# srinidhiPY/SSL_CR_Histo

Measured on AMD Instinct MI355X. Metric: images/sec (ResNet18 SSL_CR step, 256x256 bf16 synthetic patches; whole job), higher is better.
Workload: dtype bf16

## Files before the change

### include/sslcr.h

```cpp
#ifndef SSLCR_H_
#define SSLCR_H_
#include <stddef.h>
#include <stdint.h>

#ifdef __cplusplus
extern "C" {
#endif
#if defined(__GNUC__) || defined(__clang__)
#pragma GCC visibility push(default)
#endif

#define SSLCR_F32 0
#define SSLCR_BF16 1
#define SSLCR_FP8 2

int sslcr_version(void);
const char* sslcr_last_error(void);

typedef struct sslcr_conv_desc {
  const void* x;
  const void* w;
  void* y;
  const float* in_scale;
  const float* in_shift;
  const float* bias;
  const void* residual;
  float* stats;
  int N, H, W, C, K, R, S, stride, pad;
  int PH, PW;
  int OH, OW, osh;
  int transposed;
  int in_relu, relu, accumulate;
  int pix_mul, pix_off_h, pix_off_w;
  unsigned tap_mask;
  const void* mask_x; const float* mask_scale; const float* mask_shift; const float* mask_mean;
  int par4;
  int seg_images, seg_stride;
  const float* out_scale;
} sslcr_conv_desc;
int sslcr_conv2d(int dtype, const sslcr_conv_desc* d, void* stream);
int sslcr_conv2d_partial_rows(const sslcr_conv_desc* d);
int sslcr_conv2d_segments_ok(int dtype, const sslcr_conv_desc* d);
const char* sslcr_conv2d_kernel_name(int dtype, const sslcr_conv_desc* d);
int sslcr_conv2d_s2_pair(int dtype, const sslcr_conv_desc* c1, const sslcr_conv_desc* ds, void* stream);
int sslcr_conv2d_s2_pair_ok(int dtype, const sslcr_conv_desc* c1, const sslcr_conv_desc* ds);

typedef struct sslcr_fp8_desc {
  const uint8_t* w8;
  const float* w_dequant;
  float x_scale;
  const float* x_scale_dev;
  float* amax_out;
} sslcr_fp8_desc;
int sslcr_conv2d_fp8(const sslcr_conv_desc* d, const sslcr_fp8_desc* q, void* stream);
int sslcr_conv2d_fp8_partial_rows(const sslcr_conv_desc* d);
typedef struct sslcr_pack_fp8_desc {
  const float* w;
  uint8_t* w8;
  float* w_dequant;
  const float* gamma; const float* beta; const float* rmean; const float* rvar; float eps; float* bias_out;
  int K, C;
} sslcr_pack_fp8_desc;
int sslcr_pack_conv_fp8(const sslcr_pack_fp8_desc* d, void* stream);

typedef struct sslcr_wgrad_desc {
  const void* x;
  const void* dy;
  float* dw;
  const float* in_scale;
  const float* in_shift;
  int in_relu;
  int N, H, W, C, K, R, S, stride, pad, OH, OW;
  int seg_images;
  int seg_stride;
} sslcr_wgrad_desc;
int sslcr_conv2d_wgrad(int dtype, const sslcr_wgrad_desc* d, void* stream);
const char* sslcr_conv2d_wgrad_kernel_name(int dtype, const sslcr_wgrad_desc* d);

int sslcr_probe_tr16(const uint16_t* in, const int* byte_addr, uint16_t* out, void* stream);

typedef struct sslcr_stem_desc {
  const void* x;
  const void* w;
  void* y;
  const float* bias;
  float* stats;
  int N, H, W, OH, OW, in_f32, relu;
  const void* x2;
  int n_split;
  const float* out_scale;
} sslcr_stem_desc;
int sslcr_stem_conv(int dtype, const sslcr_stem_desc* d, void* stream);
int sslcr_stem_partial_rows(const sslcr_stem_desc* d);
int sslcr_stem_conv_pool(int dtype, const sslcr_stem_desc* d, int POH, int POW, void* stream);
typedef struct sslcr_stem_wgrad_desc {
  const void* x; const void* dy;
  float* dw;
  int N, H, W, OH, OW, in_f32;
  const void* x2; int n_split;
} sslcr_stem_wgrad_desc;
int sslcr_stem_wgrad(int dtype, const sslcr_stem_wgrad_desc* d, void* stream);

typedef struct sslcr_bn_finalize_desc {
  const float* partials;
  int rows, C;
  double count;
  const float* gamma; const float* beta;
  float* scale; float* shift; float* mean; float* invstd;
  float* running_mean; float* running_var; int64_t* num_batches_tracked;
  float momentum, eps; int replay;
  double* sums_out;
  const double* sums_in;
  double* stage;
  int nseg, seg_stride;
  int* tickets;
} sslcr_bn_finalize_desc;
int sslcr_bn_finalize(const sslcr_bn_finalize_desc* d, void* stream);

typedef struct sslcr_bn_act_desc {
  const void* x; const float* scale; const float* shift;
  const void* res; const float* rscale; const float* rshift;
  void* y; size_t pixels; int C; int relu;
  int nseg, seg_stride;
  uint8_t* ybits;
} sslcr_bn_act_desc;
// ... 192 lines not shown
```

### ssl_cr_histo_amd/_lib.py

```python
import ctypes as C
import os

import torch

HERE = os.path.dirname(os.path.abspath(__file__))
LIB_PATH = os.path.join(HERE, "libsslcr.so")

vp, i32, f32, f64, sz = C.c_void_p, C.c_int, C.c_float, C.c_double, C.c_size_t


class SslcrError(RuntimeError):
    pass


def _S(name, fields):
    return type(name, (C.Structure,), {"_fields_": fields})


ConvDesc = _S("ConvDesc", [("x", vp), ("w", vp), ("y", vp), ("in_scale", vp), ("in_shift", vp), ("bias", vp),
                           ("residual", vp), ("stats", vp)] +
              [(k, i32) for k in ("N", "H", "W", "C", "K", "R", "S", "stride", "pad", "PH", "PW", "OH", "OW", "osh",
                                  "transposed", "in_relu", "relu", "accumulate", "pix_mul", "pix_off_h", "pix_off_w")] +
              [("tap_mask", C.c_uint), ("mask_x", vp), ("mask_scale", vp), ("mask_shift", vp), ("mask_mean", vp),
               ("par4", i32), ("seg_images", i32), ("seg_stride", i32), ("out_scale", vp)])
WgradDesc = _S("WgradDesc", [("x", vp), ("dy", vp), ("dw", vp), ("in_scale", vp), ("in_shift", vp), ("in_relu", i32)] +
               [(k, i32) for k in ("N", "H", "W", "C", "K", "R", "S", "stride", "pad", "OH", "OW", "seg_images", "seg_stride")])
StemDesc = _S("StemDesc", [("x", vp), ("w", vp), ("y", vp), ("bias", vp), ("stats", vp)] +
              [(k, i32) for k in ("N", "H", "W", "OH", "OW", "in_f32", "relu")] + [("x2", vp), ("n_split", i32), ("out_scale", vp)])
StemWgradDesc = _S("StemWgradDesc", [("x", vp), ("dy", vp), ("dw", vp)] +
                   [(k, i32) for k in ("N", "H", "W", "OH", "OW", "in_f32")] + [("x2", vp), ("n_split", i32)])
BnFinalizeDesc = _S("BnFinalizeDesc", [("partials", vp), ("rows", i32), ("C", i32), ("count", f64), ("gamma", vp),
                                       ("beta", vp), ("scale", vp), ("shift", vp), ("mean", vp), ("invstd", vp),
                                       ("running_mean", vp), ("running_var", vp), ("num_batches_tracked", vp),
                                       ("momentum", f32), ("eps", f32), ("replay", i32), ("sums_out", vp),
                                       ("sums_in", vp), ("stage", vp), ("nseg", i32), ("seg_stride", i32), ("tickets", vp)])
BnActDesc = _S("BnActDesc", [("x", vp), ("scale", vp), ("shift", vp), ("res", vp), ("rscale", vp), ("rshift", vp),
                             ("y", vp), ("pixels", sz), ("C", i32), ("relu", i32), ("nseg", i32), ("seg_stride", i32), ("ybits", vp)])
PoolFwdDesc = _S("PoolFwdDesc", [("x", vp), ("scale", vp), ("shift", vp), ("y", vp), ("argmax", vp)] +
                 [(k, i32) for k in ("N", "H", "W", "C", "OH", "OW")])
PoolBwdDesc = _S("PoolBwdDesc", [("dy", vp), ("argmax", vp), ("x", vp), ("scale", vp), ("shift", vp), ("dx", vp)] +
                 [(k, i32) for k in ("N", "H", "W", "C", "OH", "OW")])
BnBwdDesc = _S("BnBwdDesc", [("dy", vp), ("x", vp), ("yact", vp), ("scale", vp), ("shift", vp), ("mean", vp),
                             ("invstd", vp), ("sums", vp), ("dx", vp), ("gout", vp), ("pixels", sz), ("C", i32),
                             ("relu_from_x", i32), ("count", f64), ("pool_dy", vp), ("pool_argmax", vp), ("pH", i32),
                             ("pW", i32), ("pOH", i32), ("pOW", i32), ("pool_y", vp), ("g_in_reduce", i32), ("dgamma", vp), ("dbeta", vp),
                             ("pg_scale", f32), ("nseg", i32), ("seg_stride", i32), ("sums_stride", i32), ("yact_bits", vp)])
LossDesc = _S("LossDesc", [("kind", i32), ("logits", vp), ("logits_t", vp), ("target_f", vp), ("target_i", vp),
                           ("dlogits", vp), ("out", vp), ("nx", i32), ("nu", i32), ("C", i32), ("lambda_u", f32),
                           ("inv_nx_global", f32), ("inv_nu_global", f32)])
TensorDesc = _S("TensorDesc", [("p", vp), ("g", vp), ("s1", vp), ("s2", vp), ("n", i32), ("K", i32), ("C", i32),
                               ("RS", i32), ("w_fwd", vp), ("w_dgrad", vp), ("pack_dtype", i32), ("dgrad_flip", i32)])
OptDesc = _S("OptDesc", [("kind", i32), ("lr", f32), ("beta1", f32), ("beta2", f32), ("eps", f32), ("wd", f32),
                         ("momentum", f32), ("bc1", f32), ("bc2", f32), ("first_step", i32), ("grad_scale", f32)])
WeakAugDesc = _S("WeakAugDesc", [("src", vp), ("dst", vp), ("params", vp)] +
                 [(k, i32) for k in ("N", "SH", "SW", "OH", "OW", "src_hwc")])
ColourAugDesc = _S("ColourAugDesc", [("src", vp), ("dst", vp), ("shift", vp), ("apply", vp), ("hed_from_rgb", f64 * 9),
                                     ("rgb_from_hed", f64 * 9), ("N", i32), ("H", i32), ("W", i32), ("hwc", i32)])
BrightnessContrastDesc = _S("BrightnessContrastDesc", [("src", vp), ("dst", vp), ("alpha_beta", vp), ("apply", vp), ("stats", vp),
                                                       ("N", i32), ("H", i32), ("W", i32)])
PackDesc = _S("PackDesc", [("w", vp), ("w_fwd", vp), ("w_dgrad", vp), ("gamma", vp), ("beta", vp), ("rmean", vp),
                           ("rvar", vp), ("eps", f32), ("bias_out", vp)] + [(k, i32) for k in ("K", "C", "R", "S", "dgrad_flip")] + [("scale_out", vp)])

Fp8Desc = _S("Fp8Desc", [("w8", vp), ("w_dequant", vp), ("x_scale", f32), ("x_scale_dev", vp), ("amax_out", vp)])
PackFp8Desc = _S("PackFp8Desc", [("w", vp), ("w8", vp), ("w_dequant", vp), ("gamma", vp), ("beta", vp), ("rmean", vp), ("rvar", vp),
                                 ("eps", f32), ("bias_out", vp), ("K", i32), ("C", i32)])

P = C.POINTER
SIGNATURES = {
    "sslcr_version": (i32, []),
    "sslcr_last_error": (C.c_char_p, []),
    "sslcr_conv2d": (i32, [i32, P(ConvDesc), vp]),
    "sslcr_conv2d_partial_rows": (i32, [P(ConvDesc)]),
    "sslcr_conv2d_segments_ok": (i32, [i32, P(ConvDesc)]),
    "sslcr_conv2d_kernel_name": (C.c_char_p, [i32, P(ConvDesc)]),
    "sslcr_conv2d_s2_pair": (i32, [i32, P(ConvDesc), P(ConvDesc), vp]),
    "sslcr_conv2d_s2_pair_ok": (i32, [i32, P(ConvDesc), P(ConvDesc)]),
    "sslcr_conv2d_fp8": (i32, [P(ConvDesc), P(Fp8Desc), vp]),
    "sslcr_conv2d_fp8_partial_rows": (i32, [P(ConvDesc)]),
    "sslcr_pack_conv_fp8": (i32, [P(PackFp8Desc), vp]),
    "sslcr_conv2d_wgrad": (i32, [i32, P(WgradDesc), vp]),
    "sslcr_conv2d_wgrad_kernel_name": (C.c_char_p, [i32, P(WgradDesc)]),
    "sslcr_probe_tr16": (i32, [vp, vp, vp, vp]),
    "sslcr_stem_conv": (i32, [i32, P(StemDesc), vp]),
    "sslcr_stem_partial_rows": (i32, [P(StemDesc)]),
    "sslcr_stem_conv_pool": (i32, [i32, P(StemDesc), i32, i32, vp]),
    "sslcr_stem_wgrad": (i32, [i32, P(StemWgradDesc), vp]),
    "sslcr_stem_wgrad_pool": (i32, [i32, P(StemWgradDesc), P(BnBwdDesc), vp]),
    "sslcr_bn_finalize": (i32, [P(BnFinalizeDesc), vp]),
    "sslcr_bn_act": (i32, [i32, P(BnActDesc), vp]),
    "sslcr_bn_relu_maxpool": (i32, [i32, P(PoolFwdDesc), vp]),
    "sslcr_maxpool_relu_bwd": (i32, [i32, P(PoolBwdDesc), vp]),
    "sslcr_avgpool_fwd": (i32, [i32, vp, vp, i32, i32, i32, vp]),
    "sslcr_avgpool_bwd": (i32, [i32, vp, vp, i32, i32, i32, vp]),
    "sslcr_bn_bwd_reduce": (i32, [i32, P(BnBwdDesc), vp]),
    "sslcr_bn_bwd_apply": (i32, [i32, P(BnBwdDesc), vp]),
    "sslcr_bn_param_grads": (i32, [vp, vp, vp, vp, i32, vp]),
    "sslcr_linear_fwd": (i32, [vp, vp, vp, vp, i32, i32, i32, i32, vp]),
    "sslcr_linear_bwd": (i32, [vp, vp, vp, vp, vp, vp, vp, i32, i32, i32, i32, vp, vp]),
    "sslcr_loss": (i32, [P(LossDesc), vp]),
    "sslcr_softmax_col": (i32, [vp, vp, i32, i32, i32, vp]),
    "sslcr_optimizer_step": (i32, [vp, i32, i32, P(OptDesc), vp]),
    "sslcr_axpby": (i32, [vp, vp, sz, f32, i32, vp]),
    "sslcr_fill": (i32, [vp, sz, f32, vp]),
    "sslcr_pack_conv": (i32, [i32, P(PackDesc), vp]),
    "sslcr_pack_stem": (i32, [i32, P(PackDesc), vp]),
    "sslcr_weak_augment": (i32, [P(WeakAugDesc), vp]),
    "sslcr_hed_colour_augment": (i32, [P(ColourAugDesc), vp]),
    "sslcr_brightness_contrast": (i32, [P(BrightnessContrastDesc), vp]),
}

_lib = None


def lib():
    global _lib
    if _lib is None:
        if not os.path.exists(LIB_PATH):
            raise SslcrError(f"{LIB_PATH} not built: run `python -m ssl_cr_histo_amd.build` "
                             "(or __graft_entry__.build()); there is no CPU/PyTorch fallback")
        L = C.CDLL(LIB_PATH, mode=C.RTLD_GLOBAL)
        for name, (res, args) in SIGNATURES.items():
            fn = getattr(L, name)
            fn.restype = res
            fn.argtypes = args
        _lib = L
    return _lib


def check(rc):
    if rc != 0:
        raise SslcrError(lib().sslcr_last_error().decode())


def stream_ptr():
    return C.c_void_p(torch.cuda.current_stream().cuda_stream)


def ptr(t):
    return None if t is None else C.c_void_p(t.data_ptr())
```

### ssl_cr_histo_amd/csrc/capi.cpp

```cpp
#include <stdarg.h>
#include <stdio.h>
#include <string.h>

#include "kernels.hpp"

namespace sslcr {
thread_local char g_err[512] = "";
int fail(const char* fmt, ...) {
  va_list ap;
  va_start(ap, fmt);
  vsnprintf(g_err, sizeof(g_err), fmt, ap);
  va_end(ap);
  return -1;
}
int check(hipError_t e, const char* what) {
  if (e == hipSuccess) return 0;
  return fail("%s: %s", what, hipGetErrorString(e));
}
}

using namespace sslcr;

#define NEED(cond, what) \
  do {                   \
    if (!(cond)) return fail("%s: invalid argument (%s)", __func__, what); \
  } while (0)
#define DT_OK(dt) NEED((dt) == SSLCR_F32 || (dt) == SSLCR_BF16, "dtype")

extern "C" {

int sslcr_version(void) { return 6; }
const char* sslcr_last_error(void) { return g_err; }

int sslcr_conv2d(int dtype, const sslcr_conv_desc* d, void* stream) {
  DT_OK(dtype);
  NEED(d && d->x && d->w && d->y, "null tensor");
  NEED(d->N > 0 && d->C > 0 && d->K > 0 && d->R > 0 && d->S > 0 && d->stride > 0, "shape");
  NEED(d->C % (dtype == SSLCR_BF16 ? 64 : 32) == 0, "C must be a multiple of the 128-byte channel slab");
  NEED(d->K % 64 == 0, "K % 64");
  NEED(d->osh >= 1 && d->PH > 0 && d->PW > 0, "pixel space");
  NEED(conv_segments_ok(dtype, *d), "seg_images: no segment form for this shape / dtype (sslcr_conv2d_segments_ok)");
  return check(launch_conv(dtype, *d, (hipStream_t)stream), "conv2d");
}
int sslcr_conv2d_partial_rows(const sslcr_conv_desc* d) { return d ? conv_partials_rows(*d) : -1; }
int sslcr_conv2d_segments_ok(int dtype, const sslcr_conv_desc* d) { return (d && (dtype == DT_F32 || dtype == DT_BF16) && conv_segments_ok(dtype, *d)) ? 1 : 0; }
const char* sslcr_conv2d_kernel_name(int dtype, const sslcr_conv_desc* d) { return d ? conv_kernel_name(dtype, *d) : ""; }
int sslcr_conv2d_s2_pair_ok(int dtype, const sslcr_conv_desc* c1, const sslcr_conv_desc* ds) {
  return (c1 && ds && conv_s2_pair_ok(dtype, *c1, *ds)) ? 1 : 0;
}
int sslcr_conv2d_s2_pair(int dtype, const sslcr_conv_desc* c1, const sslcr_conv_desc* ds, void* stream) {
  DT_OK(dtype);
  NEED(c1 && ds && c1->x && c1->w && c1->y && ds->w && ds->y, "null tensor");
  NEED(conv_s2_pair_ok(dtype, *c1, *ds), "pair not served (sslcr_conv2d_s2_pair_ok)");
  return check(launch_conv_s2(*c1, ds, (hipStream_t)stream), "conv2d_s2_pair");
}

int sslcr_conv2d_fp8(const sslcr_conv_desc* d, const sslcr_fp8_desc* q, void* stream) {
  NEED(d && q && d->x && d->y && q->w8 && q->w_dequant, "null tensor");
  NEED(q->x_scale > 0.f, "x_scale must be positive");
  NEED(conv_fp8_mode(*d) != 0, "shape not served by the fp8 kernel (3x3/1, C % 128, K % 128, 16x16-tileable or 8x8 with N % 4)");
  return check(launch_conv_fp8(*d, *q, (hipStream_t)stream), "conv2d_fp8");
}
int sslcr_conv2d_fp8_partial_rows(const sslcr_conv_desc* d) { return (d && conv_fp8_mode(*d)) ? conv_fp8_rows(*d) : 0; }
int sslcr_pack_conv_fp8(const sslcr_pack_fp8_desc* d, void* stream) {
  NEED(d && d->w && d->w8 && d->w_dequant && d->K > 0 && d->C > 0, "args");
  NEED(!d->gamma || (d->beta && d->rmean && d->rvar), "BatchNorm fold needs gamma, beta, running mean and var");
  return check(launch_pack_fp8(*d, (hipStream_t)stream), "pack_conv_fp8");
}

const char* sslcr_conv2d_wgrad_kernel_name(int dtype, const sslcr_wgrad_desc* d) { return d ? wgrad_kernel_name(dtype, *d) : ""; }
int sslcr_conv2d_wgrad(int dtype, const sslcr_wgrad_desc* d, void* stream) {
  DT_OK(dtype);
  NEED(d && d->x && d->dy && d->dw, "null tensor");
  NEED(d->C % 64 == 0 && d->K % 64 == 0, "C,K % 64");
  NEED((d->R == 3 && d->S == 3) || (d->R == 1 && d->S == 1), "3x3 or 1x1");
  return check(launch_wgrad(dtype, *d, (hipStream_t)stream), "conv2d_wgrad");
}

int sslcr_probe_tr16(const uint16_t* in, const int* byte_addr, uint16_t* out, void* stream) {
  NEED(in && byte_addr && out, "null");
  return check(launch_probe_tr16(in, byte_addr, out, (hipStream_t)stream), "probe_tr16");
}

int sslcr_stem_conv(int dtype, const sslcr_stem_desc* d, void* stream) {
  DT_OK(dtype);
  NEED(d && d->x && d->w && d->y, "null tensor");
  NEED(d->OH == (d->H + 6 - 7) / 2 + 1 && d->OW == (d->W + 6 - 7) / 2 + 1, "7x7/2 pad 3 output dims");
  NEED(!d->x2 || (d->n_split >= 0 && d->n_split <= d->N), "n_split outside the batch");
  return check(launch_stem(dtype, *d, (hipStream_t)stream), "stem_conv");
}
int sslcr_stem_conv_pool(int dtype, const sslcr_stem_desc* d, int POH, int POW, void* stream) {
  DT_OK(dtype);
  NEED(d && d->x && d->w && d->y, "null");
  NEED(stem_pool_ok(dtype, *d, POH, POW), "shape / mode not served by the fused stem + max-pool kernel");
  return check(launch_stem_pool(dtype, *d, POH, POW, (hipStream_t)stream), "stem_conv_pool");
}
int sslcr_stem_partial_rows(const sslcr_stem_desc* d) { return d ? stem_partials_rows(*d) : -1; }
int sslcr_stem_wgrad(int dtype, const sslcr_stem_wgrad_desc* d, void* stream) {
  DT_OK(dtype);
  NEED(d && d->x && d->dy && d->dw, "null tensor");
  NEED(!d->x2 || (d->n_split >= 0 && d->n_split <= d->N), "n_split outside the batch");
  return check(launch_stem_wgrad(dtype, *d, (hipStream_t)stream), "stem_wgrad");
}
int sslcr_stem_wgrad_pool(int dtype, const sslcr_stem_wgrad_desc* w, const sslcr_bn_bwd_desc* bn, void* stream) {
  DT_OK(dtype);
  NEED(w && w->x && w->dw && bn && bn->pool_dy && bn->pool_argmax && bn->x && bn->sums && bn->mean && bn->invstd && bn->scale && bn->shift, "null tensor");
  NEED(!w->x2 || (w->n_split >= 0 && w->n_split <= w->N), "n_split outside the batch");
  NEED(bn->C == 64 && bn->pH == w->OH && bn->pW == w->OW && bn->pixels == (size_t)w->N * w->OH * w->OW, "bn descriptor is not this stem's");
  NEED(!bn->g_in_reduce && !bn->gout, "pool form has no g output");
  return check(launch_stem_wgrad_pool(dtype, *w, *bn, (hipStream_t)stream), "stem_wgrad_pool");
}

int sslcr_bn_finalize(const sslcr_bn_finalize_desc* d, void* stream) {
  NEED(d && d->C > 0, "desc");
  NEED(d->sums_in || (d->partials && d->stage && d->rows > 0), "partials/stage");
  NEED(d->sums_out || (d->gamma && d->beta && d->scale && d->shift && d->count > 0), "finalize outputs");
  return check(launch_bn_finalize(*d, (hipStream_t)stream), "bn_finalize");
}
int sslcr_bn_act(int dtype, const sslcr_bn_act_desc* d, void* stream) {
  DT_OK(dtype);
  NEED(d && d->x && d->y && d->scale && d->shift, "null");
  NEED(d->C % 8 == 0, "C % 8");
  return check(launch_bn_act(dtype, *d, (hipStream_t)stream), "bn_act");
}
int sslcr_bn_relu_maxpool(int dtype, const sslcr_pool_fwd_desc* d, void* stream) {
  DT_OK(dtype);
  NEED(d && d->x && d->y, "null");
  if (!d->scale || !d->shift) {
    const int cols = d->C / (dtype == SSLCR_BF16 ? 8 : 4);
    NEED(!d->scale && !d->shift && !d->argmax, "plain max-pool (scale = shift = NULL) records no argmax");
    NEED(cols >= 1 && cols <= 256 && 256 % cols == 0 && d->C % (dtype == SSLCR_BF16 ? 8 : 4) == 0, "plain max-pool: unsupported channel count");
  }
  return check(launch_bn_relu_maxpool(dtype, *d, (hipStream_t)stream), "bn_relu_maxpool");
}
int sslcr_maxpool_relu_bwd(int dtype, const sslcr_pool_bwd_desc* d, void* stream) {
  DT_OK(dtype);
  NEED(d && d->x && d->dy && d->dx && d->argmax, "null");
  return check(launch_maxpool_relu_bwd(dtype, *d, (hipStream_t)stream), "maxpool_relu_bwd");
}
int sslcr_avgpool_fwd(int dtype, const void* x, float* y, int N, int HW, int C, void* stream) {
  DT_OK(dtype);
  NEED(x && y && N > 0 && HW > 0 && C % 8 == 0, "args");
// ... 83 lines not shown
```

### ssl_cr_histo_amd/csrc/common.hpp

```cpp
#pragma once
#include <hip/hip_runtime.h>
#include <stdint.h>

#include <atomic>

namespace sslcr {

typedef uint16_t bf16_t;
typedef __bf16 bf16x8_t __attribute__((ext_vector_type(8)));
typedef float f32x4_t __attribute__((ext_vector_type(4)));
typedef uint32_t u32x4_t __attribute__((ext_vector_type(4)));
typedef uint32_t u32x2_t __attribute__((ext_vector_type(2)));

enum { DT_F32 = 0, DT_BF16 = 1 };

__device__ __forceinline__ float bf2f(uint16_t v) { return __uint_as_float(((uint32_t)v) << 16); }
__device__ __forceinline__ uint16_t f2bf(float f) {
  uint32_t u = __float_as_uint(f);
  u += 0x7fffu + ((u >> 16) & 1u);
  return (uint16_t)(u >> 16);
}
__device__ __forceinline__ uint32_t pack_bf2(float lo, float hi) {
  return (uint32_t)f2bf(lo) | ((uint32_t)f2bf(hi) << 16);
}
// ... 49 lines not shown
  }
};

__device__ __forceinline__ float row16_sum(float v) {
  v += __int_as_float(__builtin_amdgcn_update_dpp(0, __float_as_int(v), 0xB1, 0xf, 0xf, true));
  v += __int_as_float(__builtin_amdgcn_update_dpp(0, __float_as_int(v), 0x4E, 0xf, 0xf, true));
  v += __int_as_float(__builtin_amdgcn_update_dpp(0, __float_as_int(v), 0x141, 0xf, 0xf, true));
  v += __int_as_float(__builtin_amdgcn_update_dpp(0, __float_as_int(v), 0x140, 0xf, 0xf, true));
  return v;
}
__device__ __forceinline__ void row16_sum4(float& a, float& b, float& c, float& d) {
  asm volatile(
      "s_nop 1\n\t"
      "v_add_f32_dpp %0, %0, %0 quad_perm:[1,0,3,2] row_mask:0xf bank_mask:0xf\n\t"
      "v_add_f32_dpp %1, %1, %1 quad_perm:[1,0,3,2] row_mask:0xf bank_mask:0xf\n\t"
      "v_add_f32_dpp %2, %2, %2 quad_perm:[1,0,3,2] row_mask:0xf bank_mask:0xf\n\t"
      "v_add_f32_dpp %3, %3, %3 quad_perm:[1,0,3,2] row_mask:0xf bank_mask:0xf\n\t"
      "v_add_f32_dpp %0, %0, %0 quad_perm:[2,3,0,1] row_mask:0xf bank_mask:0xf\n\t"
      "v_add_f32_dpp %1, %1, %1 quad_perm:[2,3,0,1] row_mask:0xf bank_mask:0xf\n\t"
      "v_add_f32_dpp %2, %2, %2 quad_perm:[2,3,0,1] row_mask:0xf bank_mask:0xf\n\t"
      "v_add_f32_dpp %3, %3, %3 quad_perm:[2,3,0,1] row_mask:0xf bank_mask:0xf\n\t"
      "v_add_f32_dpp %0, %0, %0 row_half_mirror row_mask:0xf bank_mask:0xf\n\t"
      "v_add_f32_dpp %1, %1, %1 row_half_mirror row_mask:0xf bank_mask:0xf\n\t"
      "v_add_f32_dpp %2, %2, %2 row_half_mirror row_mask:0xf bank_mask:0xf\n\t"
      "v_add_f32_dpp %3, %3, %3 row_half_mirror row_mask:0xf bank_mask:0xf\n\t"
      "v_add_f32_dpp %0, %0, %0 row_mirror row_mask:0xf bank_mask:0xf\n\t"
      "v_add_f32_dpp %1, %1, %1 row_mirror row_mask:0xf bank_mask:0xf\n\t"
      "v_add_f32_dpp %2, %2, %2 row_mirror row_mask:0xf bank_mask:0xf\n\t"
      "v_add_f32_dpp %3, %3, %3 row_mirror row_mask:0xf bank_mask:0xf"
      : "+v"(a), "+v"(b), "+v"(c), "+v"(d));
}
__device__ __forceinline__ void row16_fold16(float (&v)[16]) {
  asm volatile(
      "s_nop 1\n\t"
      "v_add_f32_dpp %0, %0, %0 row_ror:8 row_mask:0xf bank_mask:0x3\n\t"
      "v_add_f32_dpp %0, %8, %8 row_ror:8 row_mask:0xf bank_mask:0xc\n\t"
      "v_add_f32_dpp %1, %1, %1 row_ror:8 row_mask:0xf bank_mask:0x3\n\t"
      "v_add_f32_dpp %1, %9, %9 row_ror:8 row_mask:0xf bank_mask:0xc\n\t"
      "v_add_f32_dpp %2, %2, %2 row_ror:8 row_mask:0xf bank_mask:0x3\n\t"
      "v_add_f32_dpp %2, %10, %10 row_ror:8 row_mask:0xf bank_mask:0xc\n\t"
      "v_add_f32_dpp %3, %3, %3 row_ror:8 row_mask:0xf bank_mask:0x3\n\t"
      "v_add_f32_dpp %3, %11, %11 row_ror:8 row_mask:0xf bank_mask:0xc\n\t"
      "v_add_f32_dpp %4, %4, %4 row_ror:8 row_mask:0xf bank_mask:0x3\n\t"
      "v_add_f32_dpp %4, %12, %12 row_ror:8 row_mask:0xf bank_mask:0xc\n\t"
      "v_add_f32_dpp %5, %5, %5 row_ror:8 row_mask:0xf bank_mask:0x3\n\t"
      "v_add_f32_dpp %5, %13, %13 row_ror:8 row_mask:0xf bank_mask:0xc\n\t"
      "v_add_f32_dpp %6, %6, %6 row_ror:8 row_mask:0xf bank_mask:0x3\n\t"
      "v_add_f32_dpp %6, %14, %14 row_ror:8 row_mask:0xf bank_mask:0xc\n\t"
      "v_add_f32_dpp %7, %7, %7 row_ror:8 row_mask:0xf bank_mask:0x3\n\t"
      "v_add_f32_dpp %7, %15, %15 row_ror:8 row_mask:0xf bank_mask:0xc\n\t"
      "v_add_f32_dpp %0, %0, %0 row_half_mirror row_mask:0xf bank_mask:0x5\n\t"
      "v_add_f32_dpp %0, %4, %4 row_half_mirror row_mask:0xf bank_mask:0xa\n\t"
      "v_add_f32_dpp %1, %1, %1 row_half_mirror row_mask:0xf bank_mask:0x5\n\t"
      "v_add_f32_dpp %1, %5, %5 row_half_mirror row_mask:0xf bank_mask:0xa\n\t"
      "v_add_f32_dpp %2, %2, %2 row_half_mirror row_mask:0xf bank_mask:0x5\n\t"
      "v_add_f32_dpp %2, %6, %6 row_half_mirror row_mask:0xf bank_mask:0xa\n\t"
      "v_add_f32_dpp %3, %3, %3 row_half_mirror row_mask:0xf bank_mask:0x5\n\t"
      "v_add_f32_dpp %3, %7, %7 row_half_mirror row_mask:0xf bank_mask:0xa\n\t"
      "v_add_f32_dpp %0, %0, %0 quad_perm:[1,0,3,2] row_mask:0xf bank_mask:0xf\n\t"
      "v_add_f32_dpp %1, %1, %1 quad_perm:[1,0,3,2] row_mask:0xf bank_mask:0xf\n\t"
      "v_add_f32_dpp %2, %2, %2 quad_perm:[1,0,3,2] row_mask:0xf bank_mask:0xf\n\t"
      "v_add_f32_dpp %3, %3, %3 quad_perm:[1,0,3,2] row_mask:0xf bank_mask:0xf\n\t"
      "v_add_f32_dpp %0, %0, %0 quad_perm:[2,3,0,1] row_mask:0xf bank_mask:0xf\n\t"
      "v_add_f32_dpp %1, %1, %1 quad_perm:[2,3,0,1] row_mask:0xf bank_mask:0xf\n\t"
      "v_add_f32_dpp %2, %2, %2 quad_perm:[2,3,0,1] row_mask:0xf bank_mask:0xf\n\t"
      "v_add_f32_dpp %3, %3, %3 quad_perm:[2,3,0,1] row_mask:0xf bank_mask:0xf"
      : "+&v"(v[0]), "+&v"(v[1]), "+&v"(v[2]), "+&v"(v[3]), "+&v"(v[4]), "+&v"(v[5]), "+&v"(v[6]), "+&v"(v[7])
      : "v"(v[8]), "v"(v[9]), "v"(v[10]), "v"(v[11]), "v"(v[12]), "v"(v[13]), "v"(v[14]), "v"(v[15]));
}
__device__ __forceinline__ float wave_sum(float v) {
  v = row16_sum(v);
  v += __shfl_xor(v, 16);
  v += __shfl_xor(v, 32);
  return v;
}

__device__ __forceinline__ float clamp_lo(float x, float lo) { return __builtin_amdgcn_fmed3f(x, lo, __builtin_inff()); }
__device__ __forceinline__ float relu0(float x) { return __builtin_amdgcn_fmed3f(x, 0.f, __builtin_inff()); }

__device__ __forceinline__ u32x4_t ld16(const void* p) { return *reinterpret_cast<const u32x4_t*>(p); }
__device__ __forceinline__ void st16(void* p, const u32x4_t& v) { *reinterpret_cast<u32x4_t*>(p) = v; }
__device__ __forceinline__ u32x4_t ld16_nt(const void* p) { return __builtin_nontemporal_load(reinterpret_cast<const u32x4_t*>(p)); }
__device__ __forceinline__ void st16_nt(void* p, const u32x4_t& v) { __builtin_nontemporal_store(v, reinterpret_cast<u32x4_t*>(p)); }

struct LdsDma {
#if defined(__HIP_DEVICE_COMPILE__)
  __amdgpu_buffer_rsrc_t r;
#endif
  __device__ __forceinline__ void init(const void* base, unsigned bytes) {
#if defined(__HIP_DEVICE_COMPILE__)
    r = __builtin_amdgcn_make_buffer_rsrc(const_cast<void*>(base), 0, (int)bytes, 0x00020000);
#endif
  }
  __device__ __forceinline__ void load16(void* dst, int voff, int soff) const {
#if defined(__HIP_DEVICE_COMPILE__)
    __builtin_amdgcn_raw_ptr_buffer_load_lds(r, (__attribute__((address_space(3))) void*)dst, 16, voff, soff, 0, 0);
#endif
  }
};

template <int TK>
__device__ __forceinline__ int wperm(int r) {
  constexpr int B = 16 * TK;
  const int blk = r / B, x = r - blk * B;
  const int q = x / (4 * TK), y = x - q * (4 * TK);
  return blk * B + (y >> 2) * 16 + q * 4 + (y & 3);
}

static inline int cdiv(int a, int b) { return (a + b - 1) / b; }

template <typename T, int TK, int TP, bool RES, bool ACC, bool RELU, bool BIAS = true>
__device__ __forceinline__ void conv_store_tile_t(const f32x4_t (&acc)[TK][TP], const float (&bias)[4 * TK], const size_t (&off)[TP],
                                                  const bool (&ok)[TP], char* yg, const char* rg) {
  constexpr int EPC = Elem<T>::EPC, RQ = 4 * TK / EPC;
  u32x4_t r1[RES ? TP : 1][RES ? RQ : 1], r2[ACC ? TP : 1][ACC ? RQ : 1];
  if constexpr (RES) {
#pragma unroll
    for (int p = 0; p < TP; ++p)
#pragma unroll
      for (int q = 0; q < RQ; ++q) r1[p][q] = ld16(rg + off[p] + q * 16);
  }
  if constexpr (ACC) {
#pragma unroll
    for (int p = 0; p < TP; ++p)
#pragma unroll
      for (int q = 0; q < RQ; ++q) r2[p][q] = ld16(yg + off[p] + q * 16);
  }
#pragma unroll
  for (int p = 0; p < TP; ++p) {
    float v[4 * TK];
#pragma unroll
    for (int t = 0; t < TK; ++t)
#pragma unroll
      for (int j = 0; j < 4; ++j) v[t * 4 + j] = BIAS ? acc[t][p][j] + bias[t * 4 + j] : acc[t][p][j];
#pragma unroll
    for (int q = 0; q < RQ; ++q) {
      float* vq = v + q * EPC;
      if constexpr (RES) {
        float rr[EPC];
        Elem<T>::unpack(r1[p][q], rr);
#pragma unroll
        for (int e = 0; e < EPC; ++e) vq[e] += rr[e];
      }
      if constexpr (ACC) {
        float rr[EPC];
        Elem<T>::unpack(r2[p][q], rr);
#pragma unroll
        for (int e = 0; e < EPC; ++e) vq[e] += rr[e];
      }
      if constexpr (RELU) {
#pragma unroll
        for (int e = 0; e < EPC; ++e) vq[e] = relu0(vq[e]);
      }
      if (ok[p]) st16(yg + off[p] + q * 16, PackH<T>::run(vq));
    }
  }
}
template <int TK, int TP>
__device__ __forceinline__ void conv_scale_acc(f32x4_t (&acc)[TK][TP], const float* osc_kb) {
#pragma unroll
  for (int t = 0; t < TK; ++t) {
    const f32x4_t s4 = *reinterpret_cast<const f32x4_t*>(osc_kb + 4 * t);
#pragma unroll
    for (int p = 0; p < TP; ++p)
#pragma unroll
      for (int j = 0; j < 4; ++j) acc[t][p][j] *= s4[j];
// ... 24 lines not shown
```

### ssl_cr_histo_amd/csrc/conv_h16.hip

```cpp
#include "kernels.hpp"

namespace sslcr {

template <typename T> struct MmaH;
template <> struct MmaH<bf16_t> {
  __device__ static __forceinline__ void run(const u32x4_t& a, const u32x4_t& b, f32x4_t& c) {
    c = __builtin_amdgcn_mfma_f32_16x16x32_bf16(__builtin_bit_cast(bf16x8_t, a), __builtin_bit_cast(bf16x8_t, b), c, 0, 0, 0);
  }
};
template <> struct MmaH<float> {
  __device__ static __forceinline__ void run(const u32x4_t& a, const u32x4_t& b, f32x4_t& c) {
#pragma unroll
    for (int e = 0; e < 4; ++e)
      c = __builtin_amdgcn_mfma_f32_16x16x4f32(__uint_as_float(a[e]), __uint_as_float(b[e]), c, 0, 0, 0);
  }
};

template <int TK>
__device__ __forceinline__ int wperm_inv(int rr) {
  constexpr int B = 16 * TK;
  const int blk = rr / B, x = rr - blk * B;
  const int t = x >> 4, q = (x >> 2) & 3, j = x & 3;
  return blk * B + q * (4 * TK) + t * 4 + j;
}

#define SSLCR_WAIT_VM0() __builtin_amdgcn_s_waitcnt(0x0f70)
#define SSLCR_BARE_BARRIER() asm volatile("s_barrier" ::: "memory")

#ifdef SSLCR_H16_PROF
__device__ unsigned long long g_h16_prof[16][8];
#define H16_T(v) const unsigned long long v = __builtin_readcyclecounter()
#define H16_ACC(i, d) h16_t[i] += (d)
#else
#define H16_T(v)
#define H16_ACC(i, d)
#endif

template <typename T, int BKO, int WK, bool XF, bool WR, bool RAW = false, int TW = 16>
__global__ __launch_bounds__(256 * WK, WK == 1 ? 1 : 2) void conv3x3_h16_kernel(const ConvArgs a, const int tiles_total, const int n_items, const int kshift,
                                                                                const int row0) {
  constexpr bool OSC = false;
#include "conv_h16_body.hpp"
}
template <typename T, int BKO, int WK, bool WR, int TW>
__global__ __launch_bounds__(256 * WK, WK == 1 ? 1 : 2) void conv3x3_h16s_kernel(const ConvArgs a, const int tiles_total, const int n_items, const int kshift,
                                                                                 const int row0) {
  constexpr bool OSC = true, XF = false, RAW = false;
#include "conv_h16_body.hpp"
}

static int h16_mode(int dtype, const ConvArgs& a) {
  const int q = conv_halo256_mode(dtype, a);
  if (q == 16 && conv_halo256_mode(DT_BF16, a) == 16) return 16;
  static const bool on8 = [] { const char* e = getenv("SSLCR_H16_TW8"); return !e || atoi(e) != 0; }();
  if (q == 8 && on8 && conv_halo256_mode(DT_BF16, a) == 8 && a.K % 128 == 0 && !a.mask_x && (a.seg_images <= 0 || a.seg_images % 4 == 0)) return 8;
  return 0;
}
bool conv_h16_ok(int dtype, const ConvArgs& a) {
  if (a.in_scale && a.residual) return false;
  if (a.mask_x) {
    if (!a.mask_scale || !a.mask_shift || !a.mask_mean || a.in_scale || a.bias || a.residual || a.relu || a.out_scale) return false;
    if (18 * 24 * 128 + 2 * 3 * (a.K % 128 == 0 ? 128 : 64) * 128 + 2 * a.C * 4 + 8 * 128 * 4 + 3 * a.K * 4 > 160 * 1024) return false;
  }
  if (a.out_scale) {
    if (a.in_scale || a.stats || !a.bias) return false;
    const int mode = h16_mode(dtype, a);
    if (mode == 0) return false;
    const int bko = a.K % 128 == 0 ? 128 : 64;
    if (!(a.C == 64 && a.K == 64) &&
        (mode == 16 ? 18 * 24 : 4 * 10 * 10) * 128 + 2 * 3 * bko * 128 + 2 * a.C * 4 + 8 * bko * 4 + 2 * a.K * 4 > 160 * 1024) return false;
  }
  return h16_mode(dtype, a) != 0;
}
static int h16_tiles(const ConvArgs& a, int nseg) {
  return a.H == 8 ? (a.N / nseg) / 4 : (a.N / nseg) * (a.H / 16) * (a.W / 16);
}
static int h16_grid(const ConvArgs& a, int bko) {
  const int nseg = a.seg_images > 0 ? a.N / a.seg_images : 1;
  const int n_items = h16_tiles(a, nseg) * (a.K / bko);
  const int per = device_cus() / nseg;
  return (n_items < per ? n_items : per) * nseg;
}
static int h16_tail8(const ConvArgs& a) {
  if (a.H != 8 || a.seg_images > 0) return 0;
  const int cus = device_cus(), tiles = a.N / 4, kb = a.K / 128, rem = (tiles * kb) % cus;
  if (rem == 0 || 2 * rem > cus || rem % kb != 0 || tiles <= rem / kb) return 0;
  return rem / kb;
}
static ConvArgs h16_head8(const ConvArgs& a, int tail) { ConvArgs h = a; h.N = a.N - 4 * tail; return h; }
static ConvArgs h16_tailargs8(const ConvArgs& a, int tail, int dtype) {
  ConvArgs t = a;
  const int n0 = a.N - 4 * tail;
  const size_t es = dtype == DT_BF16 ? 2 : 4, px = (size_t)n0 * a.H * a.W;
  t.N = 4 * tail;
  t.x = reinterpret_cast<const char*>(a.x) + px * a.C * es;
  t.y = reinterpret_cast<char*>(a.y) + px * a.K * es;
  if (a.residual) t.residual = reinterpret_cast<const char*>(a.residual) + px * a.K * es;
  return t;
}
int conv_h16_rows(const ConvArgs& a) {
  if (a.seg_images > 0 && conv_pp64_ok(DT_BF16, a)) return conv_pp64_rows(a);
  const int tail = h16_tail8(a);
  if (tail) return (h16_grid(h16_head8(a, tail), 128) + h16_grid(h16_tailargs8(a, tail, DT_BF16), 64)) * 4;
  return h16_grid(a, a.K % 128 == 0 ? 128 : 64) * 4;
}

static bool h16_resident(const ConvArgs& a) { return a.C == 64 && a.K == 64; }
static bool h16_raw(const ConvArgs& a) {
  static const bool on = [] { const char* e = getenv("SSLCR_H16_RAW"); return !e || atoi(e) != 0; }();
  return on && a.stats && !a.bias && !a.relu && !a.residual && !a.mask_x;
}

template <typename T, int BKO, int WK, bool XF, bool WR = false, bool RAW = false, int TW = 16, bool OSC = false>
static hipError_t launch_h(const ConvArgs& a, hipStream_t st, int row0 = 0) {
  const size_t lds = (TW == 16 ? 18 * 24 : 4 * 10 * 10) * 128 + (WR ? 3 : 2) * 3 * BKO * 128 + 2 * a.C * sizeof(float) + 8 * BKO * sizeof(float) +
                     (a.mask_x ? 3 : (a.out_scale ? 2 : 1)) * a.K * sizeof(float);
  if (lds > 160 * 1024) return hipErrorInvalidValue;
  static_assert(!OSC || (!XF && !RAW), "output scale: eval forms only");
  void (*kern)(const ConvArgs, const int, const int, const int, const int);
  if constexpr (OSC) kern = conv3x3_h16s_kernel<T, BKO, WK, WR, TW>;
  else kern = conv3x3_h16_kernel<T, BKO, WK, XF, WR, RAW, TW>;
  if (OSC != (a.out_scale != nullptr)) return hipErrorInvalidValue;
  static std::atomic<bool> attr_done{false};
  if (!attr_done) {
    hipError_t e = hipFuncSetAttribute(reinterpret_cast<const void*>(kern), hipFuncAttributeMaxDynamicSharedMemorySize, 160 * 1024);
    if (e != hipSuccess) return e;
    attr_done = true;
  }
  const int nseg = a.seg_images > 0 ? a.N / a.seg_images : 1;
  const int tiles = h16_tiles(a, nseg);
  const int n_items = tiles * (a.K / BKO);
  const int grid = h16_grid(a, BKO);
  const int kbn = a.K / BKO, gseg = grid / nseg;
  const int kshift = (kbn > 1 && (kbn & (kbn - 1)) == 0 && (gseg & (kbn - 1)) == 0) ? __builtin_ctz(kbn) : -1;
  hipLaunchKernelGGL(kern, dim3(grid), dim3(256 * WK), lds, st, a, tiles, n_items, kshift, row0);
  return hipGetLastError();
}

template <typename T>
static hipError_t launch_ht8(const ConvArgs& a, hipStream_t st) {
  const bool xf = a.in_scale != nullptr;
  auto wide = [&](const ConvArgs& q) {
    if (q.out_scale) return launch_h<T, 128, 2, false, false, false, 8, true>(q, st);
    if constexpr (sizeof(T) == 2)
      if (h16_raw(q)) return xf ? launch_h<T, 128, 2, true, false, true, 8>(q, st) : launch_h<T, 128, 2, false, false, true, 8>(q, st);
    return xf ? launch_h<T, 128, 2, true, false, false, 8>(q, st) : launch_h<T, 128, 2, false, false, false, 8>(q, st);
  };
  const int tail = h16_tail8(a);
  if (!tail) return wide(a);
  const ConvArgs head = h16_head8(a, tail), tl = h16_tailargs8(a, tail, Elem<T>::DT);
  hipError_t e = wide(head);
  if (e != hipSuccess) return e;
  const int row0 = h16_grid(head, 128) * 4;
  if (tl.out_scale) return launch_h<T, 64, 2, false, false, false, 8, true>(tl, st, row0);
  return xf ? launch_h<T, 64, 2, true, false, false, 8>(tl, st, row0) : launch_h<T, 64, 2, false, false, false, 8>(tl, st, row0);
}

template <typename T>
static hipError_t launch_ht(const ConvArgs& a, hipStream_t st) {
  const bool xf = a.in_scale != nullptr;
  if (h16_mode(Elem<T>::DT, a) == 8) return launch_ht8<T>(a, st);
  if (a.K % 128 == 0) {
    if (a.out_scale) return launch_h<T, 128, 2, false, false, false, 16, true>(a, st);
    if constexpr (sizeof(T) == 2)
      if (h16_raw(a)) return xf ? launch_h<T, 128, 2, true, false, true>(a, st) : launch_h<T, 128, 2, false, false, true>(a, st);
    return xf ? launch_h<T, 128, 2, true>(a, st) : launch_h<T, 128, 2, false>(a, st);
  }
  if constexpr (sizeof(T) == 2)
    if (h16_resident(a)) {
      if (conv_pp64_ok(DT_BF16, a)) return launch_conv_pp64(a, st);
      if (a.out_scale) return launch_h<T, 64, 2, false, true, false, 16, true>(a, st);
      return xf ? launch_h<T, 64, 2, true, true>(a, st) : launch_h<T, 64, 2, false, true>(a, st);
    }
  if (a.out_scale) return launch_h<T, 64, 2, false, false, false, 16, true>(a, st);
  return xf ? launch_h<T, 64, 2, true>(a, st) : launch_h<T, 64, 2, false>(a, st);
}

hipError_t launch_conv_h16(int dtype, const ConvArgs& a, hipStream_t st) {
  if (a.mask_x && !a.stats) return hipErrorInvalidValue;
  return dtype == DT_BF16 ? launch_ht<bf16_t>(a, st) : launch_ht<float>(a, st);
// ... 32 lines not shown
```

### ssl_cr_histo_amd/csrc/conv_h16_body.hpp

```cpp
  constexpr int NT = 256 * WK;
  constexpr int EPC = Elem<T>::EPC;
  constexpr int CE = 8 * EPC;
  static_assert(TW == 16 || (TW == 8 && !WR), "tile forms");
  constexpr int TH = TW, NI = 256 / (TW * TH), HH = TH + 2, HWD = TW + 2, PITCH = TW == 16 ? 24 : 10;
  constexpr int HP = TW == 16 ? HH * HWD : 256;
  constexpr int NLD = (HP * 8 + NT - 1) / NT;
  constexpr int TK = BKO / (16 * WK), TP = 4;
  constexpr int HBUF = NI * HH * PITCH * 128, WBUF = BKO * 128, TPB = 3;
  static_assert(NLD <= 16, "staging shape");
  extern __shared__ __attribute__((aligned(16))) char smem[];
  char* s_halo = smem;
  constexpr int NRING = WR ? 3 : 2;
  char* s_w = smem + HBUF;
  float* s_scale = reinterpret_cast<float*>(smem + HBUF + NRING * TPB * WBUF);
  float* s_shift = s_scale + a.C;
  float* s_stat = s_shift + a.C;

  const int tid = threadIdx.x, lane = tid & 63;
  const int wave = __builtin_amdgcn_readfirstlane(tid >> 6);
  const int g = lane >> 4, li = lane & 15;
  const int wp = wave & 3, wk = wave >> 2;
  const int tiles_w = TW == 16 ? a.W / TW : 1, tiles_h = TW == 16 ? a.H / TH : 1;
  const int nseg = a.seg_images > 0 ? a.N / a.seg_images : 1;
  const int G = gridDim.x / nseg;
// ... 48 lines not shown
  const bool loader = WK == 1 || wave >= 4;
  constexpr int WLI = BKO / 32;
  const int lw = wave & 3;
  constexpr int WROWS = BKO / WLI;
  int wsrc0;
  {
    const int rr = lw * 8 + (lane >> 3);
    const int krow = wperm_inv<TK>(rr);
    const int c16 = (lane & 7) ^ (rr & 7);
    wsrc0 = (int)(((size_t)krow * 9 * a.C + c16 * EPC) * sizeof(T));
  }
  int Bb[3][2], Ab[2];
#pragma unroll
  for (int kk = 0; kk < 2; ++kk) {
    const int ci = kk * 4 + g;
#pragma unroll
    for (int s = 0; s < 3; ++s)
      Bb[s][kk] = TW == 16 ? ((wp * 4) * PITCH + li + s) * 128 + ((ci ^ ((li + s) & 7)) << 4)
                           : ((wp * HH + (li >> 3)) * PITCH + (li & 7) + s) * 128 + ((ci ^ (((li & 7) + s) & 7)) << 4);
    Ab[kk] = (wk * (BKO / WK) + li) * 128 + ((ci ^ (li & 7)) << 4);
  }
  const char* xg = reinterpret_cast<const char*>(a.x) + (size_t)chunk * EPC * sizeof(T);
  const char* wg = reinterpret_cast<const char*>(a.w);
  const int nslabs = a.C / CE;

  const bool kfast = kshift >= 0;
  struct Geo { int origin, k0, tile, n0, h0, w0; unsigned long long out; };
  auto geom = [&](int item) {
    Geo q;
    const int kbi = kfast ? item & ((1 << kshift) - 1) : item / tiles_total;
    q.tile = kfast ? item >> kshift : item - kbi * tiles_total;
    q.k0 = kbi * BKO;
    int t = q.tile;
    const int tw_i = t % tiles_w; t /= tiles_w;
    const int th_i = t % tiles_h;
    q.n0 = (t / tiles_h) * NI + seg_n0;
    q.h0 = th_i * TH; q.w0 = tw_i * TW;
    q.origin = (q.n0 * a.H + q.h0) * a.W + q.w0;
    q.out = TW == 8 ? 0ull : (unsigned long long)((q.h0 == 0) | ((q.h0 + TH >= a.H) << 1) | ((q.w0 == 0) << 2) | ((q.w0 + TW >= a.W) << 3)) *
                             0x1111111111111111ull;
    return q;
  };

  u32x4_t hreg[NLD];
  unsigned hin = 0;
  auto load_halo = [&](const Geo& q, int slab) {
    const unsigned long long bad = edge & q.out;
    hin = 0;
#pragma unroll
    for (int i = 0; i < NLD; ++i) {
      const bool ok = ((hvalid >> i) & 1u) && !((bad >> (4 * i)) & 0xfull);
      const int idx = q.origin + (ok ? rel[i] : 0);
      hreg[i] = ld16_nt(xg + ((size_t)idx * a.C + slab * CE) * sizeof(T));
      hin |= (ok ? 1u : 0u) << i;
    }
  };
  float sc[EPC], sh[EPC];
  auto load_affine = [&](int slab) {
    if (XF) {
      const int cb = slab * CE + chunk * EPC;
#pragma unroll
      for (int e = 0; e < EPC; ++e) { sc[e] = s_scale[cb + e]; sh[e] = s_shift[cb + e]; }
    }
  };
  auto xform_one = [&](int i) {
    u32x4_t v = hreg[i];
    if (XF) {
      float f[EPC];
      Elem<T>::unpack(v, f);
#pragma unroll
      for (int e = 0; e < EPC; ++e) f[e] = clamp_lo(fmaf(f[e], sc[e], sh[e]), relu_lo);
      v = PackH<T>::run(f);
    }
    const bool ok = (hin >> i) & 1u;
#pragma unroll
    for (int e = 0; e < 4; ++e) v[e] = ok ? v[e] : 0u;
    hreg[i] = v;
  };
  auto store_halo = [&]() {
#pragma unroll
    for (int i = 0; i < NLD; ++i)
      if ((hvalid >> i) & 1u) st16(s_halo + st_off[i], hreg[i]);
  };
  LdsDma wdma;
  wdma.init(wg, 0x7fffffffu);
  auto dma_w = [&](int k0, int slab, int tap0, int half) {
    if (!loader) return;
#pragma unroll
    for (int tt = 0; tt < TPB; ++tt) {
      const int soff = (int)(((size_t)k0 * 9 * a.C + (size_t)(tap0 + tt) * a.C + slab * CE) * sizeof(T));
#pragma unroll
      for (int i = 0; i < WLI; ++i) {
        char* dst = s_w + (half * TPB + tt) * WBUF + (i * WROWS + lw * 8) * 128;
        wdma.load16(dst, wsrc0, soff + wperm_inv<TK>(i * WROWS) * 9 * a.C * (int)sizeof(T));
      }
    }
  };

  f32x4_t acc[TK][TP];
#pragma unroll
  for (int t = 0; t < TK; ++t)
#pragma unroll
    for (int p = 0; p < TP; ++p) acc[t][p] = f32x4_t{0.f, 0.f, 0.f, 0.f};

  u32x4_t A[2][TK], B[2][TP];
  auto frags = [&](int buf, int step, const char* ringg) {
    const int tap = step >> 1, kk = step & 1;
    const int r = tap / 3, s = tap - 3 * r;
    A[buf][0] = ld16(ringg + Ab[kk] + s * WBUF);
#pragma unroll
    for (int p = 0; p < TP; ++p) B[buf][p] = ld16(s_halo + Bb[s][kk] + ((TW == 16 ? p : 2 * p) + r) * (PITCH * 128));
#pragma unroll
    for (int t = 1; t < TK; ++t) A[buf][t] = ld16(ringg + Ab[kk] + s * WBUF + t * 2048);
  };

  if (TW == 8) {
    for (int i = tid; i < HBUF / 16; i += NT) st16(s_halo + i * 16, u32x4_t{0u, 0u, 0u, 0u});
    __syncthreads();
  }
  Geo cur = geom(first);
  dma_w(cur.k0, 0, 0, 0);
  if constexpr (WR) { dma_w(cur.k0, 0, 3, 1); dma_w(cur.k0, 0, 6, 2); }
  load_halo(cur, 0);
  if (XF) __syncthreads();
  load_affine(0);
#pragma unroll
  for (int i = 0; i < NLD; ++i) xform_one(i);
  store_halo();
  SSLCR_WAIT_VM0();
  __syncthreads();
  frags(0, 0, s_w);

  char* yg = reinterpret_cast<char*>(a.y);
  const char* rg = (XF || RAW) ? nullptr : reinterpret_cast<const char*>(a.mask_x ? a.mask_x : a.residual);
  constexpr bool RPRE = sizeof(T) == 2 && !XF && !RAW;
  constexpr int RQ = 4 * TK / EPC;
  u32x4_t rres[RPRE ? TP : 1][RPRE ? RQ : 1];
  auto out_off = [&](const Geo& q, int p) {
    const int h = q.h0 + wp * 4 + p, w = q.w0 + li;
    const size_t pix = TW == 16 ? ((size_t)q.n0 * a.H + h) * a.W + w : (size_t)(q.n0 + wp) * 64 + p * 16 + li;
    return (pix * a.K + q.k0 + wk * (BKO / WK) + g * (4 * TK)) * sizeof(T);
  };
  int wb = 0, item = first, slab = 0;
  unsigned pub = 0;
#ifdef SSLCR_H16_PROF
  unsigned long long h16_t[8] = {0, 0, 0, 0, 0, 0, 0, 0};
  const unsigned long long h16_begin = __builtin_readcyclecounter();
#endif
  for (;;) {
    const bool last = slab + 1 == nslabs;
    const bool done = last && item + G >= n_items;
    const int nslab = last ? 0 : slab + 1;
    const Geo nxt = (last && !done) ? geom(item + G) : cur;
    const char* ring0 = s_w + wb * (TPB * WBUF);
    const char* ring1 = s_w + (wb ^ 1) * (TPB * WBUF);

    auto load_res = [&]() {
      if constexpr (RPRE) {
        if (rg && last) {
#pragma unroll
          for (int p = 0; p < TP; ++p)
#pragma unroll
            for (int q = 0; q < RQ; ++q) rres[p][q] = ld16(rg + out_off(cur, p) + q * 16);
        }
      }
    };
    if constexpr (WR) {
      load_res();
      load_halo(nxt, 0);
    } else {
      dma_w(cur.k0, slab, 3, wb ^ 1);
    }
    __builtin_amdgcn_sched_barrier(0);
#pragma unroll
    for (int i = 0; i < 18; ++i) {
      if (i < 17) frags((i + 1) & 1, i + 1, WR ? s_w + ((i + 1) / 6) * (TPB * WBUF) : ((((i + 1) / 6) & 1) ? ring1 : ring0));
      if (sizeof(T) != 2) __builtin_amdgcn_sched_barrier(0);
#pragma unroll
      for (int t = 0; t < TK; ++t)
#pragma unroll
        for (int p = 0; p < TP; ++p) MmaH<T>::run(A[i & 1][t], B[i & 1][p], acc[t][p]);
      if (i < 17 && sizeof(T) == 2) {
#pragma unroll
        for (int q = 0; q < TK + TP; ++q) {
          __builtin_amdgcn_sched_group_barrier(0x100, 1, 0);
          __builtin_amdgcn_sched_group_barrier(0x008, (TK * TP) / (TK + TP), 0);
        }
      }
      if (i >= 15) {
#pragma unroll
        for (int j = (i - 15); j < NLD; j += 3) xform_one(j);
      }
      __builtin_amdgcn_sched_barrier(0);
      if (WR && i == 14) {
        SSLCR_WAIT_VM0();
        __builtin_amdgcn_sched_barrier(0);
      }
      if (!WR && i % 6 == 2) {
        H16_T(tp0);
        SSLCR_WAIT_VM0();
        H16_T(tp1);
        SSLCR_BARE_BARRIER();
        H16_T(tp2);
        H16_ACC(0, tp1 - tp0); H16_ACC(1, tp2 - tp1);
        if (i == 8) {
          load_res();
          load_halo(nxt, nslab);
          load_affine(nslab);
        }
        __builtin_amdgcn_sched_barrier(0);
      }
      if (!WR && (i == 5 || i == 11)) {
        H16_T(tf0);
        SSLCR_BARE_BARRIER();
        H16_T(tf1);
        H16_ACC(2, tf1 - tf0);
        if (i == 5) dma_w(cur.k0, slab, 6, wb); else dma_w(nxt.k0, nslab, 0, wb ^ 1);
        __builtin_amdgcn_sched_barrier(0);
      }
    }
    H16_T(ts0);
    SSLCR_BARE_BARRIER();
    store_halo();
    __syncthreads();
    H16_T(ts1);
    H16_ACC(3, ts1 - ts0); H16_ACC(5, 1);
    wb ^= 1;
    frags(0, 0, WR ? s_w : s_w + wb * (TPB * WBUF));
    __builtin_amdgcn_sched_barrier(0);

    H16_T(te0);
    if (last) {
      const int kb = cur.k0 + wk * (BKO / WK) + g * (4 * TK);
      float s1[4 * TK], s2[4 * TK];
      if (mk) {
#pragma unroll
        for (int q = 0; q < 4 * TK / EPC; ++q) {
          float msc[EPC], msh[EPC], mmu[EPC], a1[EPC], a2[EPC];
#pragma unroll
          for (int e = 0; e < EPC; ++e) {
            msc[e] = s_bias[kb + q * EPC + e]; msh[e] = s_msh[kb + q * EPC + e]; mmu[e] = s_mmu[kb + q * EPC + e];
            a1[e] = 0.f; a2[e] = 0.f;
          }
#pragma unroll
          for (int p = 0; p < TP; ++p) {
            const size_t off = out_off(cur, p);
            float xr[EPC], vq[EPC];
            if constexpr (RPRE) Elem<T>::unpack(rres[p][q], xr);
            else Elem<T>::unpack(ld16(rg + off + q * 16), xr);
#pragma unroll
            for (int e = 0; e < EPC; ++e) {
              const int idx = q * EPC + e;
              const float y = acc[idx >> 2][p][idx & 3];
              const float gv = fmaf(xr[e], msc[e], msh[e]) > 0.f ? y : 0.f;
              vq[e] = gv;
              a1[e] += gv;
              a2[e] = fmaf(gv, xr[e] - mmu[e], a2[e]);
            }
            st16(yg + off + q * 16, PackH<T>::run(vq));
          }
#pragma unroll
          for (int e = 0; e < EPC; ++e) { s1[q * EPC + e] = a1[e]; s2[q * EPC + e] = a2[e]; }
        }
      } else {
      if constexpr (RAW) {
#pragma unroll
        for (int p = 0; p < TP; ++p) {
          const size_t off = out_off(cur, p);
#pragma unroll
          for (int q = 0; q < 4 * TK / EPC; ++q) {
            float vq[EPC];
#pragma unroll
            for (int e = 0; e < EPC; ++e) vq[e] = acc[(q * EPC + e) >> 2][p][(q * EPC + e) & 3];
            st16(yg + off + q * 16, PackH<T>::run(vq));
          }
        }
      } else if constexpr (OSC) {
#pragma unroll
      for (int q = 0; q < 4 * TK / EPC; ++q) {
        float bq[EPC], sq[EPC];
#pragma unroll
        for (int e = 0; e < EPC; ++e) { bq[e] = s_bias[kb + q * EPC + e]; sq[e] = s_osc[kb + q * EPC + e]; }
#pragma unroll
        for (int p = 0; p < TP; ++p) {
          const size_t off = out_off(cur, p);
          float vq[EPC];
#pragma unroll
          for (int e = 0; e < EPC; ++e) {
            const int idx = q * EPC + e;
            vq[e] = fmaf(acc[idx >> 2][p][idx & 3], sq[e], bq[e]);
          }
          if (rg) {
            float rr[EPC];
            if constexpr (RPRE) Elem<T>::unpack(rres[p][q], rr);
            else Elem<T>::unpack(ld16(rg + off + q * 16), rr);
#pragma unroll
            for (int e = 0; e < EPC; ++e) vq[e] += rr[e];
          }
#pragma unroll
          for (int e = 0; e < EPC; ++e) vq[e] = clamp_lo(vq[e], out_lo);
          st16(yg + off + q * 16, PackH<T>::run(vq));
        }
      }
      } else {
      float bias[4 * TK];
#pragma unroll
      for (int j = 0; j < 4 * TK; ++j) bias[j] = s_bias[kb + j];
#pragma unroll
      for (int p = 0; p < TP; ++p) {
        const size_t off = out_off(cur, p);
        float v[4 * TK];
#pragma unroll
// ... 114 lines not shown
```

### ssl_cr_histo_amd/csrc/conv_igemm.hip

```cpp
#include "kernels.hpp"

namespace sslcr {

template <typename T> struct Mma;
template <> struct Mma<bf16_t> {
  __device__ static __forceinline__ void run(const u32x4_t& a, const u32x4_t& b, f32x4_t& c) {
    c = __builtin_amdgcn_mfma_f32_16x16x32_bf16(__builtin_bit_cast(bf16x8_t, a), __builtin_bit_cast(bf16x8_t, b), c, 0, 0, 0);
  }
};
template <> struct Mma<float> {
  __device__ static __forceinline__ void run(const u32x4_t& a, const u32x4_t& b, f32x4_t& c) {
#pragma unroll
    for (int e = 0; e < 4; ++e)
      c = __builtin_amdgcn_mfma_f32_16x16x4f32(__uint_as_float(a[e]), __uint_as_float(b[e]), c, 0, 0, 0);
  }
};

template <typename T, int BP, int BKO>
__global__ __launch_bounds__(256) void conv_igemm_kernel(const ConvArgs a) {
  constexpr int EPC = Elem<T>::EPC;
  constexpr int CE = 8 * EPC;
  constexpr int TP = BP / 32;
  constexpr int TK = BKO / 32;
  constexpr int PR = BP / 32;
// ... 232 lines not shown
int conv_partials_rows(const ConvArgs& a) {
  if (conv_h16_ok(g_conv_dtype_hint, a)) return conv_h16_rows(a);
  const int q = conv_halo256_mode(g_conv_dtype_hint, a);
  if (q) return conv_halo256_tiles(a, q) * 4;
  const int tw = conv_halo_tw(g_conv_dtype_hint, a);
  if (tw) return conv_halo_tiles(a, tw) * 2;
  const int bp = conv_dma_bp(g_conv_dtype_hint, a);
  if (bp) return conv_dma_rows(a, bp);
  const int M = a.N * a.PH * a.PW;
  return cdiv(M, conv_tile_bp(a)) * 2;
}

int conv_tile_bp(const ConvArgs& a) {
  const int M = a.N * a.PH * a.PW;
  return M >= 128 * 512 ? 128 : 64;
}

template <typename T>
static hipError_t launch_t(const ConvArgs& a, hipStream_t st) {
  constexpr int CE = 8 * Elem<T>::EPC;
  if (a.C % CE != 0 || a.K % 64 != 0) return hipErrorInvalidValue;
  const int bp = conv_tile_bp(a);
  if (bp == 128) {
    if (a.K % 128 == 0) return launch_cfg<T, 128, 128>(a, st);
    return launch_cfg<T, 128, 64>(a, st);
  }
  return launch_cfg<T, 64, 64>(a, st);
}

const char* conv_kernel_name(int dtype, const ConvArgs& a) {
  const bool bf = dtype == DT_BF16;
  const bool wide = a.K % 128 == 0;
  if (conv_h16_ok(dtype, a)) return conv_h16_name(dtype, a);
  const int q = conv_halo256_mode(dtype, a);
  if (q && conv_halo256_mode(DT_BF16, a) == q) {
    const bool one = a.C == (bf ? 64 : 32);
    if (q == 16) {
      if (wide) return bf ? "sslcr::conv3x3_halo256_kernel<unsigned short, 16, 128, 2, false>" : "sslcr::conv3x3_halo256_kernel<float, 16, 128, 2, false>";
      if (one) return bf ? "sslcr::conv3x3_halo256_kernel<unsigned short, 16, 64, 1, true>" : "sslcr::conv3x3_halo256_kernel<float, 16, 64, 1, true>";
      return bf ? "sslcr::conv3x3_halo256_kernel<unsigned short, 16, 64, 2, false>" : "sslcr::conv3x3_halo256_kernel<float, 16, 64, 2, false>";
    }
    if (wide) return bf ? "sslcr::conv3x3_halo256_kernel<unsigned short, 8, 128, 2, false>" : "sslcr::conv3x3_halo256_kernel<float, 8, 128, 2, false>";
    if (one) return bf ? "sslcr::conv3x3_halo256_kernel<unsigned short, 8, 64, 1, true>" : "sslcr::conv3x3_halo256_kernel<float, 8, 64, 1, true>";
    return bf ? "sslcr::conv3x3_halo256_kernel<unsigned short, 8, 64, 2, false>" : "sslcr::conv3x3_halo256_kernel<float, 8, 64, 2, false>";
  }
  const int tw = q ? 0 : conv_halo_tw(dtype, a);
  if (tw && conv_halo_tw(DT_BF16, a) == tw) return bf ? "sslcr::conv3x3_halo_kernel<unsigned short, ...>" : "sslcr::conv3x3_halo_kernel<float, ...>";
  if (!q && !tw && conv_s2_ok(dtype, a)) return conv_s2_name(a, false);
  if (!q && !tw && conv_s2d_ok(dtype, a)) return conv_s2d_name();
  const int dbp = (q || tw) ? 0 : conv_dma_bp(dtype, a);
  if (dbp && conv_dma_bp(DT_BF16, a) == dbp) return conv_dma_name(dtype, dbp);
  const int bp = conv_tile_bp(a);
  if (bp == 128) {
    if (wide) return bf ? "sslcr::conv_igemm_kernel<unsigned short, 128, 128>" : "sslcr::conv_igemm_kernel<float, 128, 128>";
    return bf ? "sslcr::conv_igemm_kernel<unsigned short, 128, 64>" : "sslcr::conv_igemm_kernel<float, 128, 64>";
  }
  return bf ? "sslcr::conv_igemm_kernel<unsigned short, 64, 64>" : "sslcr::conv_igemm_kernel<float, 64, 64>";
}

int device_cus() {
  static const int cus = [] {
    int dev = 0, n = 0;
    if (hipGetDevice(&dev) != hipSuccess || hipDeviceGetAttribute(&n, hipDeviceAttributeMultiprocessorCount, dev) != hipSuccess || n <= 0) n = 256;
    return n;
  }();
  return cus;
}

bool conv_segments_ok(int dtype, const ConvArgs& a) {
  if (a.seg_images <= 0) return true;
  if (dtype != DT_BF16 || a.N % a.seg_images != 0 || a.transposed || a.par4) return false;
  const int nseg = a.N / a.seg_images;
  if (nseg > 8) return false;
  if (conv_h16_ok(dtype, a)) return true;
  if (a.mask_x) return false;
  const int q = conv_halo256_mode(dtype, a);
  if (q) return q == 16 || a.seg_images % 4 == 0;
  if (conv_halo_tw(dtype, a)) return false;
  const int bp = conv_dma_bp(dtype, a);
  if (bp) return !a.in_scale && ((long)a.seg_images * a.PH * a.PW) % bp == 0;
  return false;
}

hipError_t launch_conv(int dtype, const ConvArgs& a, hipStream_t st) {
  if (!conv_segments_ok(dtype, a)) return hipErrorInvalidValue;
  if (a.out_scale && (!a.bias || a.stats || a.mask_x)) return hipErrorInvalidValue;
  if (conv_h16_ok(dtype, a)) return launch_conv_h16(dtype, a, st);
  if (a.mask_x) return hipErrorInvalidValue;
  const int q = conv_halo256_mode(dtype, a);
  if (q && conv_halo256_mode(DT_BF16, a) == q) return launch_conv_halo256(dtype, a, q, st);
  const int tw = q ? 0 : conv_halo_tw(dtype, a);
  if (tw && conv_halo_tw(DT_BF16, a) == tw) return launch_conv_halo(dtype, a, tw, st);
  if (!q && !tw && conv_s2_ok(dtype, a)) return launch_conv_s2(a, nullptr, st);
  if (!q && !tw && conv_s2d_ok(dtype, a)) return launch_conv_s2d(a, st);
  const int dbp = (q || tw) ? 0 : conv_dma_bp(dtype, a);
  if (dbp && conv_dma_bp(DT_BF16, a) == dbp) return launch_conv_dma(dtype, a, dbp, st);
  if (a.par4) return hipErrorInvalidValue;
  return dtype == DT_BF16 ? launch_t<bf16_t>(a, st) : launch_t<float>(a, st);
}

}
```

### ssl_cr_histo_amd/csrc/conv_pp64.hip

```cpp
#include <stdlib.h>

#include "kernels.hpp"

namespace sslcr {

typedef const __attribute__((address_space(1))) void* gptr_pp;
typedef __attribute__((address_space(3))) void* lptr_pp;

#define SSLCR_PP_BAR() asm volatile("s_waitcnt lgkmcnt(0)\n\ts_barrier" ::: "memory")

#ifdef SSLCR_PP_PROF
__device__ unsigned long long g_pp_prof[8][8];
#define PP_T(v) const unsigned long long v = __builtin_readcyclecounter()
#define PP_ACC(i, d) pp_t[i] += (d)
#else
#define PP_T(v)
#define PP_ACC(i, d)
#endif

#define PP_CH(t, g, j) ((((t) >> 1) * 32) + ((g) * 8) + (((t) & 1) * 4) + (j))
__device__ __forceinline__ int pp_row_kout(int rr) {
  const int t = rr >> 4, gq = (rr >> 2) & 3, j = rr & 3;
  return PP_CH(t, gq, j);
}
// ... 36 lines not shown
  const int nst = (tiles_total - first0 + 2 * G - 1) / (2 * G);
  constexpr bool mk = OP == 2;
  const float relu_lo = a.in_relu ? 0.f : -__builtin_inff();

  {
    const int rr = wave * 8 + (lane >> 3);
    const int krow = pp_row_kout(rr);
    const int c16 = (lane & 7) ^ (rr & 7);
    const char* wg = reinterpret_cast<const char*>(a.w) + ((size_t)krow * 9 * 64 + c16 * EPC) * sizeof(T);
#pragma unroll
    for (int tt = 0; tt < 9; ++tt)
      __builtin_amdgcn_global_load_lds((gptr_pp)(wg + (size_t)tt * 64 * sizeof(T)), (lptr_pp)(s_w + tt * WBUF + (wave * 8) * 128), 16, 0, 0);
  }
  if (tid < 64) {
    if (XF) { s_scale[tid] = a.in_scale[(size_t)seg * a.seg_stride + tid]; s_shift[tid] = a.in_shift[(size_t)seg * a.seg_stride + tid]; }
    const size_t mo = (size_t)seg * a.seg_stride + tid;
    s_bias[tid] = mk ? a.mask_scale[mo] : (a.bias ? a.bias[tid] : 0.f);
    if (mk) { s_msh[tid] = a.mask_shift[mo]; s_mmu[tid] = a.mask_mean[mo]; }
    else if (a.out_scale) s_msh[tid] = a.out_scale[tid];
  }
  const bool osc_on = !mk && !XF && a.out_scale != nullptr;
  for (int i = tid; i < 1024; i += 512) s_f[320 + i] = 0.f;

  const int chunk = gtid & 7;
  int role[NLD];
  const int rel_bias = a.W + 1;
  unsigned long long edge = 0;
  unsigned hvalid = 0;
#pragma unroll
  for (int i = 0; i < NLD; ++i) {
    const int sp = (gtid >> 3) + (GT / 8) * i;
    role[i] = rel_bias;
    if (sp < HP) {
      const int hr = sp / HWD, hc = sp - hr * HWD;
      role[i] = ((hr - 1) * a.W + hc - 1 + rel_bias) | ((((hr * PITCH + hc) * 128 + ((chunk ^ (hc & 7)) << 4)) >> 4) << 16);
      hvalid |= 1u << i;
      edge |= (unsigned long long)((hr == 0) | ((hr == HH - 1) << 1) | ((hc == 0) << 2) | ((hc == HWD - 1) << 3)) << (4 * i);
    }
  }
  int Bb[3][2], Ab[2];
#pragma unroll
  for (int kk = 0; kk < 2; ++kk) {
    const int ci = kk * 4 + g;
#pragma unroll
    for (int s = 0; s < 3; ++s) Bb[s][kk] = ((wq * 4) * PITCH + li + s) * 128 + ((ci ^ ((li + s) & 7)) << 4);
    Ab[kk] = li * 128 + ((ci ^ (li & 7)) << 4);
  }
  const char* xg = reinterpret_cast<const char*>(a.x) + (size_t)chunk * EPC * sizeof(T);

  struct Geo { int origin, n0, h0, w0; unsigned long long out; };
  auto geom = [&](int tile) {
    Geo q;
    int t = tile;
    const int tw_i = t % tiles_w; t /= tiles_w;
    const int th_i = t % tiles_h;
    q.n0 = t / tiles_h + seg_n0;
    q.h0 = th_i * TH; q.w0 = tw_i * TW;
    q.origin = (q.n0 * a.H + q.h0) * a.W + q.w0;
    q.out = (unsigned long long)((q.h0 == 0) | ((q.h0 + TH >= a.H) << 1) | ((q.w0 == 0) << 2) | ((q.w0 + TW >= a.W) << 3)) *
            0x1111111111111111ull;
    return q;
  };
  auto tile_of = [&](int k, bool& live) {
    const int t = first0 + grp + k * 2 * G;
    live = t < tiles_total;
    return live ? t : tiles_total - 1;
  };

  u32x4_t hreg[NLD];
  unsigned hin = 0;
  auto load_halo = [&](const Geo& q) {
    const unsigned long long bad = edge & q.out;
    hin = 0;
#pragma unroll
    for (int i = 0; i < NLD; ++i) {
      const bool ok = ((hvalid >> i) & 1u) && !((bad >> (4 * i)) & 0xfull);
      int rl = role[i];
      asm volatile("" : "+v"(rl));
      const int idx = q.origin + (ok ? (rl & 0xffff) - rel_bias : 0);
      hreg[i] = ld16_nt(xg + (unsigned)idx * (unsigned)(64 * sizeof(T)));
      hin |= (ok ? 1u : 0u) << i;
    }
  };
  auto xform_store = [&]() {
    float sc[EPC], sh[EPC];
    if (XF) {
      const f32x4_t c0 = *reinterpret_cast<const f32x4_t*>(s_scale + chunk * EPC), c1 = *reinterpret_cast<const f32x4_t*>(s_scale + chunk * EPC + 4);
      const f32x4_t h0 = *reinterpret_cast<const f32x4_t*>(s_shift + chunk * EPC), h1 = *reinterpret_cast<const f32x4_t*>(s_shift + chunk * EPC + 4);
#pragma unroll
      for (int e = 0; e < 4; ++e) { sc[e] = c0[e]; sc[4 + e] = c1[e]; sh[e] = h0[e]; sh[4 + e] = h1[e]; }
    }
#pragma unroll
    for (int i = 0; i < NLD; ++i) {
      u32x4_t v = hreg[i];
      if (XF) {
        float f[EPC];
        Elem<T>::unpack(v, f);
#pragma unroll
        for (int e = 0; e < EPC; ++e) f[e] = __builtin_amdgcn_fmed3f(fmaf(f[e], sc[e], sh[e]), relu_lo, __builtin_inff());
        v = PackH<T>::run(f);
      }
      const bool ok = (hin >> i) & 1u;
#pragma unroll
      for (int e = 0; e < 4; ++e) v[e] = ok ? v[e] : 0u;
      int rl = role[i];
      asm volatile("" : "+v"(rl));
      if ((hvalid >> i) & 1u) st16(s_halo + ((rl >> 12) & 0xffff0), v);
    }
  };

  char* yg = reinterpret_cast<char*>(a.y);
  const char* rg = OP == 0 ? nullptr : reinterpret_cast<const char*>(OP == 2 ? a.mask_x : a.residual);
  u32x4_t rres[RPRE ? TP : 1][RPRE ? RQ : 1];
  auto out_off = [&](const Geo& q, int p) {
    const int h = q.h0 + wq * 4 + p, w = q.w0 + li;
    return (unsigned)(((q.n0 * a.H + h) * a.W + w) * 64 + g * 8) * (unsigned)sizeof(T);
  };
  auto load_res = [&](const Geo& q) {
    if constexpr (RPRE) {
#pragma unroll
      for (int p = 0; p < TP; ++p)
#pragma unroll
        for (int qq = 0; qq < RQ; ++qq) rres[p][qq] = ld16(rg + out_off(q, p) + qq * 64);
    }
  };

  f32x4_t acc[TK][TP];
  u32x4_t A[2][TK], B[2][TP];
  auto frags = [&](int buf, int step) {
    const int tap = step >> 1, kk = step & 1;
    const int r = tap / 3, s = tap - 3 * r;
#pragma unroll
    for (int t = 0; t < TK; ++t) A[buf][t] = ld16(s_w + Ab[kk] + tap * WBUF + t * 2048);
#pragma unroll
    for (int p = 0; p < TP; ++p) B[buf][p] = ld16(s_halo + Bb[s][kk] + (p + r) * (PITCH * 128));
  };

  bool live = false, live_n = false;
  Geo cur = geom(tile_of(0, live));
  load_halo(cur);
  __builtin_amdgcn_s_waitcnt(0x0f70);
  SSLCR_PP_BAR();
  xform_store();
  Geo nxt = geom(tile_of(1, live_n));
  load_halo(nxt);
  SSLCR_PP_BAR();
  if (grp == 1) SSLCR_PP_BAR();

#ifdef SSLCR_PP_PROF
  unsigned long long pp_t[8] = {0, 0, 0, 0, 0, 0, 0, 0};
#endif
  for (int st = 0; st < nst; ++st) {
    PP_T(t0);
    frags(0, 0);
    __builtin_amdgcn_sched_barrier(0);
#pragma unroll
    for (int i = 0; i < 18; ++i) {
      if (i < 17) frags((i + 1) & 1, i + 1);
#pragma unroll
      for (int t = 0; t < TK; ++t)
#pragma unroll
        for (int p = 0; p < TP; ++p) {
          const bf16x8_t av = __builtin_bit_cast(bf16x8_t, A[i & 1][t]), bv = __builtin_bit_cast(bf16x8_t, B[i & 1][p]);
          if (i == 0) acc[t][p] = __builtin_amdgcn_mfma_f32_16x16x32_bf16(av, bv, f32x4_t{0.f, 0.f, 0.f, 0.f}, 0, 0, 0);
          else acc[t][p] = __builtin_amdgcn_mfma_f32_16x16x32_bf16(av, bv, acc[t][p], 0, 0, 0);
        }
      if (i < 17) {
#pragma unroll
        for (int q = 0; q < TK + TP; ++q) {
          __builtin_amdgcn_sched_group_barrier(0x100, 1, 0);
          __builtin_amdgcn_sched_group_barrier(0x008, (TK * TP) / (TK + TP), 0);
        }
      }
      __builtin_amdgcn_sched_barrier(0);
    }
    PP_T(t1);
    SSLCR_PP_BAR();
    PP_T(t2);
    PP_ACC(0, t1 - t0); PP_ACC(1, t2 - t1);

    load_res(cur);
    xform_store();
    PP_T(ta);
    PP_ACC(4, ta - t2);
    {
      const int kb = g * 8;
      float s1[4 * TK], s2[4 * TK];
      if constexpr (mk) {
#pragma unroll
        for (int q = 0; q < RQ; ++q) {
          float msc[EPC], msh[EPC], mmu[EPC], a1[EPC], a2[EPC];
#pragma unroll
          for (int e = 0; e < EPC; ++e) {
            msc[e] = s_bias[kb + q * 32 + e]; msh[e] = s_msh[kb + q * 32 + e]; mmu[e] = s_mmu[kb + q * 32 + e];
            a1[e] = 0.f; a2[e] = 0.f;
          }
#pragma unroll
          for (int p = 0; p < TP; ++p) {
            float xr[EPC], vq[EPC];
            Elem<T>::unpack(rres[RPRE ? p : 0][RPRE ? q : 0], xr);
#pragma unroll
            for (int e = 0; e < EPC; ++e) {
              const int idx = q * EPC + e;
              const float y = acc[idx >> 2][p][idx & 3];
              const float gv = fmaf(xr[e], msc[e], msh[e]) > 0.f ? y : 0.f;
              vq[e] = gv;
              a1[e] += gv;
              a2[e] = fmaf(gv, xr[e] - mmu[e], a2[e]);
            }
            if (live) st16(yg + out_off(cur, p) + q * 64, PackH<T>::run(vq));
          }
#pragma unroll
          for (int e = 0; e < EPC; ++e) { s1[q * EPC + e] = a1[e]; s2[q * EPC + e] = a2[e]; }
        }
      } else {
        if (live) {
          if (OP == 0 && !a.bias && !a.relu) {
#pragma unroll
            for (int p = 0; p < TP; ++p)
#pragma unroll
              for (int q = 0; q < RQ; ++q) {
                float vq[EPC];
#pragma unroll
                for (int e = 0; e < EPC; ++e) vq[e] = acc[(q * EPC + e) >> 2][p][e & 3];
                st16(yg + out_off(cur, p) + q * 64, PackH<T>::run(vq));
              }
          } else {
            if (osc_on) {
#pragma unroll
              for (int j = 0; j < 4 * TK; ++j) {
                const float sj = s_msh[kb + (j >> 3) * 32 + (j & 7)];
#pragma unroll
                for (int p = 0; p < TP; ++p) acc[j >> 2][p][j & 3] *= sj;
              }
            }
            float bias[4 * TK];
#pragma unroll
            for (int j = 0; j < 4 * TK; ++j) bias[j] = s_bias[kb + (j >> 3) * 32 + (j & 7)];
            const float lo = a.relu ? 0.f : -__builtin_inff();
#pragma unroll
            for (int p = 0; p < TP; ++p)
#pragma unroll
              for (int q = 0; q < RQ; ++q) {
                float vq[EPC], rr[EPC];
                if constexpr (OP == 1) Elem<T>::unpack(rres[RPRE ? p : 0][RPRE ? q : 0], rr);
#pragma unroll
                for (int e = 0; e < EPC; ++e) {
                  float v = acc[(q * EPC + e) >> 2][p][e & 3] + bias[q * EPC + e];
                  if constexpr (OP == 1) v += rr[e];
                  vq[e] = __builtin_amdgcn_fmed3f(v, lo, __builtin_inff());
                }
                st16(yg + out_off(cur, p) + q * 64, PackH<T>::run(vq));
              }
          }
        }
        if (a.stats) {
#pragma unroll
          for (int t = 0; t < TK; ++t)
#pragma unroll
            for (int j = 0; j < 4; ++j) {
              float x1 = 0.f, x2 = 0.f;
#pragma unroll
              for (int p = 0; p < TP; ++p) { float q = acc[t][p][j]; x1 += q; x2 = fmaf(q, q, x2); }
              s1[t * 4 + j] = x1;
              s2[t * 4 + j] = x2;
// ... 97 lines not shown
```

### ssl_cr_histo_amd/csrc/engine.cpp

```cpp
#include <rccl/rccl.h>
#include <stdio.h>
#include <stdlib.h>
#include <string.h>

#include <atomic>
#include <chrono>
#include <condition_variable>
#include <mutex>
#include <vector>

#include "kernels.hpp"

using namespace sslcr;

#define TRY(expr)                                   \
  do {                                              \
    hipError_t _e = (expr);                         \
    if (_e != hipSuccess) return check(_e, #expr);  \
  } while (0)
#define TRYI(expr)            \
  do {                        \
    int _r = (expr);          \
    if (_r != 0) return _r;   \
  } while (0)
#define TRYN(expr)                                                                     \
  do {                                                                                 \
    ncclResult_t _r = (expr);                                                          \
    if (_r != ncclSuccess) return fail("%s: %s", #expr, ncclGetErrorString(_r));       \
  } while (0)

namespace {

struct DevBuf {
  void* p = nullptr;
  size_t cap = 0;
  int ensure(size_t bytes) {
    if (bytes <= cap) return 0;
    if (p) {
      hipError_t e = hipFree(p);
      if (e != hipSuccess) return check(e, "hipFree");
      p = nullptr;
      cap = 0;
    }
    bytes = (bytes + 255) & ~(size_t)255;
    hipError_t e = hipMalloc(&p, bytes);
    if (e != hipSuccess) return check(e, "hipMalloc");
    cap = bytes;
    return 0;
  }
  void release() {
    if (p) (void)hipFree(p);
    p = nullptr;
    cap = 0;
  }
};

struct Carver {
  size_t off = 0;
  size_t take(size_t bytes) {
    size_t o = off;
    off += (bytes + 255) & ~(size_t)255;
    return o;
  }
};

struct ConvL {
  int cin = 0, cout = 0, k = 0, stride = 1, pad = 0, pidx = -1;
  void *w_fwd = nullptr, *w_dg = nullptr, *w_fold = nullptr;
  float* b_fold = nullptr;
  float* s_fold = nullptr;
  void* w_foldf = nullptr;
  uint8_t *w8_fwd = nullptr, *w8_fold = nullptr;
  float *dq_fwd = nullptr, *dq_fold = nullptr;
  float* f8s = nullptr;
};
struct BnL {
  int C = 0, pg = -1, pb = -1, bidx = -1;
};
struct BlockL {
  ConvL c1, c2, ds;
  BnL b1, b2, bd;
  bool has_ds = false;
  int pstart = 0;
};
struct BnSaved {
  float *scale, *shift, *mean, *invstd;
};
struct PassState {
  const void* x = nullptr;
  const void* x2 = nullptr;
  int n_split = 0;
  int in_f32 = 0, N = 0, H = 0, W = 0;
  DevBuf mem;
  char* raw0 = nullptr;
  char* pooled = nullptr;
  uint8_t* argmax = nullptr;
  struct {
    char *raw1, *raw2, *rawd, *y;
    uint8_t* ybits;
  } blk[8];
  BnSaved bn[20];
  float* E = nullptr;
};

}

struct ProfRec {
  hipEvent_t e0, e1;
  double flops, bytes;
  const char* name;
};
struct Profiler {
  bool on = false;
  std::vector<ProfRec> rec[3];
  std::vector<hipEvent_t> pool;
  hipEvent_t get() {
    if (!pool.empty()) { hipEvent_t e = pool.back(); pool.pop_back(); return e; }
    hipEvent_t e = nullptr;
    (void)hipEventCreate(&e);
    return e;
  }
};

constexpr int VW_MAX = 8;
struct VChan {
  std::mutex m;
  std::condition_variable cv;
  int arrived = 0;
  long gen = 0;
  void* slot[2][VW_MAX] = {};
  size_t cap[2][VW_MAX] = {};
  hipEvent_t ev_in[2][VW_MAX] = {}, ev_out[2][VW_MAX] = {};
  bool out_set[2][VW_MAX] = {};
  long calls[VW_MAX] = {};
};
struct sslcr_vcomm {
  int world = 1;
  VChan ch[2];
  std::atomic<bool> poisoned{false};
};

struct sslcr_ctx {
  Profiler prof;
  int device = 0, dtype = 0;
  int fp8 = 0;
  sslcr_vcomm* vcomm = nullptr;
  ncclComm_t comm = nullptr;
  ncclComm_t comm_g = nullptr;
  int rank = 0, world = 1;
  int bn_sync = 1;
  hipStream_t comm_stream = nullptr;
  hipStream_t aux_stream = nullptr;
  hipEvent_t ev_aux_begin = nullptr, ev_aux_end = nullptr;
  int use_aux = 0;
  hipStream_t wg_stream = nullptr;
  hipEvent_t ev_wg_in[3] = {nullptr, nullptr, nullptr}, ev_wg_done[3] = {nullptr, nullptr, nullptr}, ev_wg_join = nullptr;
  bool wg_pending[3] = {false, false, false};
  bool wg_any = false;
  int fuse_stem_bwd = 1;
  int use_wg = 0;
  hipEvent_t ev_ready[8], ev_done = nullptr;
  DevBuf scratch;
  DevBuf partials;
  DevBuf small;
  double* bn_stage = nullptr;
  double* bn_sums = nullptr;
  int* bn_tickets = nullptr;
  DevBuf bn_ring;
  int bn_ring_i = 0;
  static constexpr int kBnRing = 96, kBnSlot = 2 * 2 * 512;
  float *ones = nullptr, *zeros = nullptr;
  size_t esz() const { return dtype == DT_BF16 ? 2 : 4; }
};

struct sslcr_net {
  sslcr_ctx* ctx = nullptr;
  const void* split_x2 = nullptr;
  int split_n = 0;
  int nparams = 0, head_kind = 0, ncls = 1, triplet = 0;
  std::vector<float*> params;
  std::vector<uint8_t> rg;
  std::vector<int> psize;
// ... 28 lines not shown
  std::vector<float*> st1, st2;
  int ndesc = 0, max_n = 0;
};

namespace {

struct VSrc { const void* p[VW_MAX]; };
template <typename T>
__global__ void vsum_kernel(T* dst, VSrc src, int W, size_t n) {
  for (size_t i = (size_t)blockIdx.x * blockDim.x + threadIdx.x; i < n; i += (size_t)gridDim.x * blockDim.x) {
    T s = static_cast<const T*>(src.p[0])[i];
    for (int q = 1; q < W; ++q) s += static_cast<const T*>(src.p[q])[i];
    dst[i] = s;
  }
}

std::atomic<int> g_live_ctx{0};

inline bool sharded(const sslcr_ctx* c) { return c->comm != nullptr || c->vcomm != nullptr; }

int vcomm_all_reduce(sslcr_ctx* c, int chan, void* buf, size_t count, bool f64, hipStream_t st) {
  sslcr_vcomm* v = c->vcomm;
  VChan& ch = v->ch[chan];
  const int r = c->rank, W = v->world;
  const size_t bytes = count * (f64 ? 8 : 4);
  if (v->poisoned) return fail("virtual all-reduce: the communicator was poisoned by an earlier timeout");
  const int ph = (int)(ch.calls[r]++ & 1);
  for (int q = 0; q < W; ++q)
    if (q != r && ch.out_set[ph][q]) TRY(hipStreamWaitEvent(st, ch.ev_out[ph][q], 0));
  if (ch.cap[ph][r] < bytes) {
    if (ch.slot[ph][r]) TRY(hipFree(ch.slot[ph][r]));
    ch.slot[ph][r] = nullptr; ch.cap[ph][r] = 0;
    TRY(hipMalloc(&ch.slot[ph][r], (bytes + 255) & ~(size_t)255));
    ch.cap[ph][r] = (bytes + 255) & ~(size_t)255;
  }
  if (!ch.ev_in[ph][r]) {
    TRY(hipEventCreateWithFlags(&ch.ev_in[ph][r], hipEventDisableTiming));
    TRY(hipEventCreateWithFlags(&ch.ev_out[ph][r], hipEventDisableTiming));
  }
  TRY(hipMemcpyAsync(ch.slot[ph][r], buf, bytes, hipMemcpyDeviceToDevice, st));
  TRY(hipEventRecord(ch.ev_in[ph][r], st));
  {
    std::unique_lock<std::mutex> lk(ch.m);
    const long g = ch.gen;
    if (++ch.arrived == W) {
      ch.arrived = 0; ++ch.gen;
      ch.cv.notify_all();
    } else if (!ch.cv.wait_for(lk, std::chrono::seconds(120), [&] { return ch.gen != g; })) {
      --ch.arrived;
      c->vcomm->poisoned = true;
      ch.cv.notify_all();
      return fail("virtual all-reduce: rank %d waited 120 s for its peers (channel %d); the communicator is now unusable", r, chan);
    }
  }
  VSrc src;
  for (int q = 0; q < W; ++q) {
    src.p[q] = ch.slot[ph][q];
    if (q != r) TRY(hipStreamWaitEvent(st, ch.ev_in[ph][q], 0));
  }
  const int blocks = (int)((count + 255) / 256 < 1024 ? (count + 255) / 256 : 1024);
  if (f64) hipLaunchKernelGGL(vsum_kernel<double>, dim3(blocks), dim3(256), 0, st, (double*)buf, src, W, count);
  else hipLaunchKernelGGL(vsum_kernel<float>, dim3(blocks), dim3(256), 0, st, (float*)buf, src, W, count);
  TRY(hipGetLastError());
  TRY(hipEventRecord(ch.ev_out[ph][r], st));
  ch.out_set[ph][r] = true;
  return 0;
}

int all_reduce(sslcr_ctx* c, int chan, void* buf, size_t count, bool f64, hipStream_t st) {
  if (c->vcomm) return vcomm_all_reduce(c, chan, buf, count, f64, st);
  TRYN(ncclAllReduce(buf, buf, count, f64 ? ncclDouble : ncclFloat, ncclSum, chan == 0 ? c->comm : c->comm_g, st));
  return 0;
}

hipError_t prof_conv(sslcr_ctx* c, int dt, const ConvArgs& a, hipStream_t st) {
  if (!c->prof.on) return launch_conv(dt, a, st);
  ProfRec r;
  r.e0 = c->prof.get(); r.e1 = c->prof.get();
  const double es = c->esz();
  const double rs = a.tap_mask ? (double)__builtin_popcount(a.tap_mask) : (double)a.R * a.S;
  const double M = (double)a.N * a.PH * a.PW;
  const double src = (double)a.N * a.H * a.W;
  r.flops = a.transposed ? 2.0 * src * a.C * a.K * rs : 2.0 * M * a.K * a.C * rs;
  r.bytes = (src * a.C + (double)a.K * rs * a.C + M * a.K * (a.residual ? 2.0 : 1.0) * (a.accumulate ? 2.0 : 1.0)) * es;
  r.name = conv_kernel_name(dt, a);
  (void)hipEventRecord(r.e0, st);
  hipError_t e = launch_conv(dt, a, st);
  (void)hipEventRecord(r.e1, st);
  c->prof.rec[0].push_back(r);
  return e;
}
hipError_t prof_conv_pair(sslcr_ctx* c, const ConvArgs& a, const ConvArgs& d, hipStream_t st) {
  if (!c->prof.on) return launch_conv_s2(a, &d, st);
  ProfRec r;
  r.e0 = c->prof.get(); r.e1 = c->prof.get();
  const double es = c->esz();
  const double M = (double)a.N * a.PH * a.PW, src = (double)a.N * a.H * a.W;
  r.flops = 2.0 * M * a.K * a.C * 10.0;
  r.bytes = (src * a.C + (double)a.K * 10.0 * a.C + 2.0 * M * a.K) * es;
  r.name = conv_s2_name(a, true);
  (void)hipEventRecord(r.e0, st);
  hipError_t e = launch_conv_s2(a, &d, st);
  (void)hipEventRecord(r.e1, st);
  c->prof.rec[0].push_back(r);
  return e;
}
inline bool fp8_layer(const sslcr_ctx* c, const ConvL& L) {
  return c->fp8 && L.k == 3 && L.stride == 1 && L.cin % 128 == 0 && L.cout % 128 == 0;
}
inline bool use_fp8(const sslcr_ctx* c, const ConvL& L, const ConvArgs& a) { return fp8_layer(c, L) && L.w8_fwd && conv_fp8_mode(a) != 0; }
hipError_t prof_conv_fwd(sslcr_ctx* c, int dt, const ConvArgs& a_in, const ConvL& L, bool folded, hipStream_t st) {
  ConvArgs a = a_in;
  a.out_scale = nullptr;
  if (!use_fp8(c, L, a)) return prof_conv(c, dt, a_in, st);
  Fp8Args q;
  q.w8 = folded ? L.w8_fold : L.w8_fwd;
  q.w_dequant = folded ? L.dq_fold : L.dq_fwd;
  q.x_scale = 1.0f;
  q.x_scale_dev = L.f8s ? L.f8s + (folded ? 2 : 0) : nullptr;
  q.amax_out = L.f8s ? L.f8s + (folded ? 3 : 1) : nullptr;
  if (!c->prof.on) return launch_conv_fp8(a, q, st);
  ProfRec r;
  r.e0 = c->prof.get(); r.e1 = c->prof.get();
  const double M = (double)a.N * a.PH * a.PW;
  r.flops = 2.0 * M * a.K * a.C * 9.0;
  r.bytes = ((double)a.N * a.H * a.W * a.C + M * a.K * (a.residual ? 2.0 : 1.0)) * 2.0 + (double)a.K * 9.0 * a.C;
  r.name = conv_fp8_name(a);
  (void)hipEventRecord(r.e0, st);
  hipError_t e = launch_conv_fp8(a, q, st);
  (void)hipEventRecord(r.e1, st);
  c->prof.rec[0].push_back(r);
  return e;
}
hipError_t prof_wgrad(sslcr_ctx* c, int dt, const WgradArgs& a, hipStream_t st) {
  if (!c->prof.on) return launch_wgrad(dt, a, st);
  ProfRec r;
  r.e0 = c->prof.get(); r.e1 = c->prof.get();
  const double es = c->esz();
  const double M = (double)a.N * a.OH * a.OW;
  r.flops = 2.0 * M * a.K * a.C * a.R * a.S;
  r.bytes = ((double)a.N * a.H * a.W * a.C + M * a.K) * es + (double)a.K * a.R * a.S * a.C * 4.0;
  r.name = wgrad_kernel_name(dt, a);
  (void)hipEventRecord(r.e0, st);
  hipError_t e = launch_wgrad(dt, a, st);
  (void)hipEventRecord(r.e1, st);
  c->prof.rec[1].push_back(r);
  return e;
}

constexpr int kMaxSeg = 3;
const int kBlockCfg[8][3] ={{64, 64, 1}, {64, 64, 1}, {64, 128, 2}, {128, 128, 1}, {128, 256, 2}, {256, 256, 1}, {256, 512, 2}, {512, 512, 1}};

inline int out_dim(int h, int k, int stride, int pad) { return (h + 2 * pad - k) / stride + 1; }

void build_topology(sslcr_net* n) {
  int p = 0, b = 0;
  n->stem = ConvL{3, 64, 7, 2, 3, p++};
  n->bn0 = BnL{64, p, p + 1, b++};
  p += 2;
  for (int i = 0; i < 8; ++i) {
    BlockL& B = n->blocks[i];
    const int cin = kBlockCfg[i][0], cout = kBlockCfg[i][1], s = kBlockCfg[i][2];
    B.pstart = p;
    B.c1 = ConvL{cin, cout, 3, s, 1, p++};
    B.b1 = BnL{cout, p, p + 1, b++};
    p += 2;
    B.c2 = ConvL{cout, cout, 3, 1, 1, p++};
// ... 164 lines not shown
  a.tickets = c->bn_tickets;
  if (sharded(c) && c->bn_sync) {
    BnFinalizeArgs r = a;
    r.sums_out = c->bn_sums;
    TRY(launch_bn_finalize(r, st));
    TRYI(all_reduce(c, 0, c->bn_sums, 2 * (size_t)bn.C, true, st));
    a.sums_in = c->bn_sums;
    a.count = local_count * c->world;
  } else {
    a.count = local_count;
  }
  TRY(launch_bn_finalize(a, st));
  return 0;
}

int finalize_bn_pair(sslcr_net* n, const BnL& b1, const float* part1, int rows1, const BnL& bd, const float* partd, int rowsd, double local_count,
                     BnSaved& sv1, BnSaved& svd, int replay, hipStream_t st, int nseg, int seg_stride) {
  sslcr_ctx* c = n->ctx;
  if (!(sharded(c) && c->bn_sync) || b1.C != bd.C || nseg > 1) {
    TRYI(finalize_bn(n, b1, part1, rows1, local_count, sv1, replay, st, nseg, seg_stride));
    return finalize_bn(n, bd, partd, rowsd, local_count, svd, replay, st, nseg, seg_stride);
  }
  const BnL* bns[2] = {&b1, &bd};
  const float* parts[2] = {part1, partd};
  const int rowsv[2] = {rows1, rowsd};
  BnSaved* svs[2] = {&sv1, &svd};
  BnFinalizeArgs a[2];
  for (int i = 0; i < 2; ++i) {
    memset(&a[i], 0, sizeof(a[i]));
    a[i].partials = parts[i]; a[i].rows = rowsv[i]; a[i].C = bns[i]->C;
    a[i].gamma = n->params[bns[i]->pg]; a[i].beta = n->params[bns[i]->pb];
    a[i].scale = svs[i]->scale; a[i].shift = svs[i]->shift; a[i].mean = svs[i]->mean; a[i].invstd = svs[i]->invstd;
    a[i].running_mean = n->bn_rm[bns[i]->bidx]; a[i].running_var = n->bn_rv[bns[i]->bidx]; a[i].num_batches_tracked = n->bn_nbt[bns[i]->bidx];
    if (n->f8_calib_pass) { a[i].running_mean = nullptr; a[i].running_var = nullptr; a[i].num_batches_tracked = nullptr; }
    a[i].momentum = 0.1f; a[i].eps = 1e-5f; a[i].replay = replay;
    a[i].stage = c->bn_stage; a[i].tickets = c->bn_tickets;
    BnFinalizeArgs r = a[i];
    r.sums_out = c->bn_sums + (size_t)i * 2 * b1.C;
    TRY(launch_bn_finalize(r, st));
  }
  TRYI(all_reduce(c, 0, c->bn_sums, 4 * (size_t)b1.C, true, st));
  for (int i = 0; i < 2; ++i) {
    a[i].sums_in = c->bn_sums + (size_t)i * 2 * b1.C;
    a[i].count = local_count * c->world;
    TRY(launch_bn_finalize(a[i], st));
  }
  return 0;
}

ConvArgs conv_args(const ConvL& L, const void* x, const void* w, void* y, int N, int H, int W) {
  ConvArgs a;
  memset(&a, 0, sizeof(a));
  a.x = x; a.w = w; a.y = y;
  a.N = N; a.H = H; a.W = W; a.C = L.cin; a.K = L.cout; a.R = L.k; a.S = L.k; a.stride = L.stride; a.pad = L.pad;
  a.PH = out_dim(H, L.k, L.stride, L.pad); a.PW = out_dim(W, L.k, L.stride, L.pad);
  a.OH = a.PH; a.OW = a.PW; a.osh = 1;
  return a;
}

int ensure_partials(sslcr_ctx* c, const ConvArgs& a, float** out, int* rows, bool fp8 = false) {
  *rows = fp8 ? conv_fp8_rows(a) : conv_partials_rows(a);
  TRYI(c->partials.ensure((size_t)*rows * 2 * a.K * sizeof(float)));
  *out = (float*)c->partials.p;
  return 0;
}

struct Dims {
  int oh0, ow0, ph, pw;
  int lh[8], lw[8];
};
Dims make_dims(int H, int W) {
  Dims d;
  d.oh0 = out_dim(H, 7, 2, 3); d.ow0 = out_dim(W, 7, 2, 3);
  d.ph = out_dim(d.oh0, 3, 2, 1); d.pw = out_dim(d.ow0, 3, 2, 1);
  int h = d.ph, w = d.pw;
  for (int i = 0; i < 8; ++i) {
    const int s = kBlockCfg[i][2];
    h = out_dim(h, 3, s, 1); w = out_dim(w, 3, s, 1);
    d.lh[i] = h; d.lw[i] = w;
  }
  return d;
}

int alloc_passes(sslcr_net* n, int npass, int N, int H, int W) {
  const size_t es = n->ctx->esz();
  const Dims d = make_dims(H, W);
  Carver c;
  auto take = [&](size_t per_pass) { return c.take(per_pass * npass); };
  const size_t s_raw0 = (size_t)N * d.oh0 * d.ow0 * 64 * es, s_pool = (size_t)N * d.ph * d.pw * 64 * es, s_arg = (size_t)N * d.ph * d.pw * 64;
  const size_t o_raw0 = take(s_raw0), o_pool = take(s_pool), o_arg = take(s_arg);
  size_t o_blk[8][4], s_blk[8], o_bits[8], s_bits[8];
  bool bits_ok = true;
  for (int i = 0; i < 8; ++i) {
    s_blk[i] = (size_t)N * d.lh[i] * d.lw[i] * kBlockCfg[i][1] * es;
    for (int j = 0; j < 4; ++j) o_blk[i][j] = (j == 2 && !n->blocks[i].has_ds) ? 0 : take(s_blk[i]);
    s_bits[i] = (((size_t)N * d.lh[i] * d.lw[i] * kBlockCfg[i][1] / 8) + 127) / 128 * 128;
    o_bits[i] = take(s_bits[i]);
    if (s_bits[i] * 8 != (size_t)N * d.lh[i] * d.lw[i] * kBlockCfg[i][1]) bits_ok = false;
  }
  const size_t s_bn = 20 * 4 * 512 * sizeof(float), s_E = (size_t)N * 512 * sizeof(float);
  const size_t o_bn = take(s_bn), o_E = take(s_E);
  TRYI(n->pass[0].mem.ensure(c.off));
  char* b = (char*)n->pass[0].mem.p;
  for (int p = 0; p < npass; ++p) {
    PassState& ps = n->pass[p];
    ps.raw0 = b + o_raw0 + p * s_raw0; ps.pooled = b + o_pool + p * s_pool; ps.argmax = (uint8_t*)(b + o_arg + p * s_arg);
    for (int i = 0; i < 8; ++i) {
      ps.blk[i].raw1 = b + o_blk[i][0] + p * s_blk[i]; ps.blk[i].raw2 = b + o_blk[i][1] + p * s_blk[i];
      ps.blk[i].rawd = n->blocks[i].has_ds ? b + o_blk[i][2] + p * s_blk[i] : nullptr;
      ps.blk[i].y = b + o_blk[i][3] + p * s_blk[i];
      ps.blk[i].ybits = (uint8_t*)(b + o_bits[i] + p * s_bits[i]);
    }
    float* f = (float*)(b + o_bn + p * s_bn);
    for (int i = 0; i < 20; ++i) {
      ps.bn[i] = BnSaved{f, f + 512, f + 1024, f + 1536};
      f += 2048;
    }
    ps.E = (float*)(b + o_E + p * s_E);
    ps.N = N; ps.H = H; ps.W = W;
  }
  n->ybits_ok = bits_ok;
  return 0;
}

int forward_stem(sslcr_net* n, PassState& ps, const void* x, int in_f32, int N, int H, int W, int replay, hipStream_t st) {
  sslcr_ctx* c = n->ctx;
  const int dt = c->dtype;
  const Dims d = make_dims(H, W);
  ps.x = x; ps.in_f32 = in_f32;
  StemArgs a;
  memset(&a, 0, sizeof(a));
  a.x = x; a.x2 = ps.x2; a.n_split = ps.n_split; a.w = n->stem.w_fwd; a.y = ps.raw0;
  a.N = N; a.H = H; a.W = W; a.OH = d.oh0; a.OW = d.ow0; a.in_f32 = in_f32;
  const int rows = stem_partials_rows(a);
  TRYI(c->partials.ensure((size_t)rows * 2 * 64 * sizeof(float)));
  a.stats = (float*)c->partials.p;
  TRY(launch_stem(dt, a, st));
  TRYI(finalize_bn(n, n->bn0, a.stats, rows, (double)N * d.oh0 * d.ow0, ps.bn[0], replay, st));
  PoolFwdArgs p;
  memset(&p, 0, sizeof(p));
  p.x = ps.raw0; p.scale = ps.bn[0].scale; p.shift = ps.bn[0].shift; p.y = ps.pooled; p.argmax = ps.argmax;
  p.N = N; p.H = d.oh0; p.W = d.ow0; p.C = 64; p.OH = d.ph; p.OW = d.pw;
  TRY(launch_bn_relu_maxpool(dt, p, st));
  return 0;
}

bool ybits_on(const sslcr_ctx* c) {
  static const bool on = [] { const char* e = getenv("SSLCR_YBITS"); return !e || atoi(e) != 0; }();
  return on && c->dtype == DT_BF16;
}
const uint8_t* ybits_of(const sslcr_net* n, const void* yact) {
  if (!yact || !n->ybits_ok || !ybits_on(n->ctx)) return nullptr;
  for (int p = 0; p < 3; ++p)
    for (int i = 0; i < 8; ++i)
      if (n->pass[p].blk[i].y == yact) return n->pass[p].blk[i].ybits;
  return nullptr;
}

int forward_blocks(sslcr_net* n, PassState& ps, int N, int H, int W, int replay, int nseg, hipStream_t st) {
  sslcr_ctx* c = n->ctx;
  const int dt = c->dtype;
  const Dims d = make_dims(H, W);
  const bool segs = nseg > 1;
  const int NT = nseg * N;
  const int seg_stride = segs ? (int)(n->pass[1].bn[0].scale - n->pass[0].bn[0].scale) : 0;
  const char* X = ps.pooled;
  int xh = d.ph, xw = d.pw;
  for (int i = 0; i < 8; ++i) {
    BlockL& B = n->blocks[i];
    const int oh = d.lh[i], ow = d.lw[i];
    const double cnt = (double)N * oh * ow;
    float* part; int rows;
    ConvArgs a1 = conv_args(B.c1, X, B.c1.w_fwd, ps.blk[i].raw1, NT, xh, xw);
    if (segs) a1.seg_images = N;
    ConvArgs ad;
    bool paired = false;
    if (B.has_ds) {
      ad = conv_args(B.ds, X, B.ds.w_fwd, ps.blk[i].rawd, NT, xh, xw);
      if (segs) ad.seg_images = N;
      ConvArgs t1 = a1, td = ad;
      t1.stats = td.stats = c->zeros;
      paired = !use_fp8(c, B.c1, a1) && conv_s2_pair_ok(dt, t1, td);
    }
    if (paired) {
      if (segs && (!conv_segments_ok(dt, a1) || !conv_segments_ok(dt, ad))) return fail("forward_blocks: the paired stride-2 launch has no segment form here");
      rows = conv_partials_rows(a1);
      const size_t rb = (size_t)rows * 2 * a1.K * sizeof(float);
      TRYI(c->partials.ensure(2 * rb));
      part = (float*)c->partials.p;
      a1.stats = part;
      ad.stats = (float*)((char*)c->partials.p + rb);
      TRY(prof_conv_pair(c, a1, ad, st));
      TRYI(finalize_bn_pair(n, B.b1, a1.stats, rows, B.bd, ad.stats, rows, cnt, ps.bn[B.b1.bidx], ps.bn[B.bd.bidx], replay, st, nseg, seg_stride));
    } else if (B.has_ds) {
      const int rows1 = conv_partials_rows(a1), rowsd = conv_partials_rows(ad);
      const size_t rb1 = (((size_t)rows1 * 2 * a1.K * sizeof(float)) + 255) & ~(size_t)255;
      TRYI(c->partials.ensure(rb1 + (size_t)rowsd * 2 * ad.K * sizeof(float)));
      a1.stats = (float*)c->partials.p;
      ad.stats = (float*)((char*)c->partials.p + rb1);
      TRY(prof_conv(c, dt, a1, st));
      TRY(prof_conv(c, dt, ad, st));
      TRYI(finalize_bn_pair(n, B.b1, a1.stats, rows1, B.bd, ad.stats, rowsd, cnt, ps.bn[B.b1.bidx], ps.bn[B.bd.bidx], replay, st, nseg, seg_stride));
      paired = true;
    } else {
      TRYI(ensure_partials(c, a1, &part, &rows, !segs && use_fp8(c, B.c1, a1)));
      a1.stats = part;
      TRY(segs ? prof_conv(c, dt, a1, st) : prof_conv_fwd(c, dt, a1, B.c1, false, st));
      TRYI(finalize_bn(n, B.b1, part, rows, cnt, ps.bn[B.b1.bidx], replay, st, nseg, seg_stride));
    }
    ConvArgs a2 = conv_args(B.c2, ps.blk[i].raw1, B.c2.w_fwd, ps.blk[i].raw2, NT, oh, ow);
    a2.in_scale = ps.bn[B.b1.bidx].scale; a2.in_shift = ps.bn[B.b1.bidx].shift; a2.in_relu = 1;
    if (segs) { a2.seg_images = N; a2.seg_stride = seg_stride; }
    TRYI(ensure_partials(c, a2, &part, &rows, !segs && use_fp8(c, B.c2, a2)));
    a2.stats = part;
    TRY(segs ? prof_conv(c, dt, a2, st) : prof_conv_fwd(c, dt, a2, B.c2, false, st));
    TRYI(finalize_bn(n, B.b2, part, rows, cnt, ps.bn[B.b2.bidx], replay, st, nseg, seg_stride));
    BnActArgs e;
    memset(&e, 0, sizeof(e));
    e.x = ps.blk[i].raw2; e.scale = ps.bn[B.b2.bidx].scale; e.shift = ps.bn[B.b2.bidx].shift;
    e.y = ps.blk[i].y; e.pixels = (size_t)NT * oh * ow; e.C = B.c2.cout; e.relu = 1;
    if (segs) { e.nseg = nseg; e.seg_stride = seg_stride; }
    if (n->ybits_ok && ybits_on(c)) e.ybits = ps.blk[i].ybits;
    if (B.has_ds) {
      if (!paired) {
        TRYI(ensure_partials(c, ad, &part, &rows));
        ad.stats = part;
        TRY(prof_conv(c, dt, ad, st));
        TRYI(finalize_bn(n, B.bd, part, rows, cnt, ps.bn[B.bd.bidx], replay, st, nseg, seg_stride));
      }
      e.res = ps.blk[i].rawd; e.rscale = ps.bn[B.bd.bidx].scale; e.rshift = ps.bn[B.bd.bidx].shift;
    } else {
      e.res = X;
    }
    TRY(launch_bn_act(dt, e, st));
    X = ps.blk[i].y; xh = oh; xw = ow;
  }
  TRY(launch_avgpool_fwd(dt, X, ps.E, NT, xh * xw, 512, st));
  return 0;
}

int backbone_forward_train(sslcr_net* n, PassState& ps, const void* x, int in_f32, int N, int H, int W, int replay, hipStream_t st) {
  if (n->pass[0].N != N || n->pass[0].H != H || n->pass[0].W != W || !n->pass[0].mem.p) TRYI(alloc_passes(n, n->triplet ? 3 : 1, N, H, W));
  ps.x2 = n->split_x2; ps.n_split = n->split_x2 ? n->split_n : 0;
  TRYI(forward_stem(n, ps, x, in_f32, N, H, W, replay, st));
  return forward_blocks(n, ps, N, H, W, replay, 1, st);
}

bool segments_on() {
  static const bool on = [] { const char* e = getenv("SSLCR_SEGMENTS"); return !(e && e[0] == '0'); }();
  return on;
}
bool segments_servable(sslcr_net* n, int N, int H, int W) {
  sslcr_ctx* c = n->ctx;
  if (!segments_on() || !n->triplet || c->dtype != DT_BF16 || c->fp8 || (sharded(c) && c->bn_sync) || c->prof.on) return false;
  const Dims d = make_dims(H, W);
  int xh = d.ph, xw = d.pw;
  for (int i = 0; i < 8; ++i) {
    BlockL& B = n->blocks[i];
    const int oh = d.lh[i], ow = d.lw[i];
    ConvArgs a1 = conv_args(B.c1, nullptr, nullptr, nullptr, 3 * N, xh, xw);
    a1.seg_images = N;
    ConvArgs a2 = conv_args(B.c2, nullptr, nullptr, nullptr, 3 * N, oh, ow);
    a2.seg_images = N; a2.in_scale = c->ones; a2.in_shift = c->zeros;
    if (!conv_segments_ok(c->dtype, a1) || !conv_segments_ok(c->dtype, a2)) return false;
    if (B.has_ds) {
      ConvArgs ad = conv_args(B.ds, nullptr, nullptr, nullptr, 3 * N, xh, xw);
      ad.seg_images = N;
      if (!conv_segments_ok(c->dtype, ad)) return false;
    }
    if (conv_partials_rows(a1) % 3 || conv_partials_rows(a2) % 3) return false;
    xh = oh; xw = ow;
  }
  return true;
}

int backbone_forward_train_segments(sslcr_net* n, const void* const* xs, int in_f32, int N, int H, int W, hipStream_t st) {
  constexpr int NS = 3;
  if (n->pass[0].N != N || n->pass[0].H != H || n->pass[0].W != W || !n->pass[0].mem.p) TRYI(alloc_passes(n, NS, N, H, W));
  for (int p = 0; p < NS; ++p) {
    n->pass[p].x2 = nullptr; n->pass[p].n_split = 0;
    TRYI(forward_stem(n, n->pass[p], xs[p], in_f32, N, H, W, 1, st));
  }
  return forward_blocks(n, n->pass[0], N, H, W, 1, NS, st);
}

int backbone_forward_eval(sslcr_net* n, const void* const* xs, int npass, int in_f32, int N, int H, int W, float* const* E, hipStream_t st) {
  sslcr_ctx* c = n->ctx;
  const int dt = c->dtype;
  const size_t es = c->esz();
  const Dims d = make_dims(H, W);
  const int NT = npass * N;
  Carver cv;
  const size_t o_a0 = cv.take((size_t)N * d.oh0 * d.ow0 * 64 * es);
  const size_t unit1 = (size_t)N * d.ph * d.pw * 64 * es, unit = unit1 * npass;
  size_t o_buf[4];
  for (int j = 0; j < 4; ++j) o_buf[j] = cv.take(unit);
  TRYI(c->scratch.ensure(cv.off));
// ... 261 lines not shown
  sslcr_ctx* c = n->ctx;
  WgradArgs a;
  memset(&a, 0, sizeof(a));
  a.x = x; a.dy = dy; a.dw = (float*)n->grads.p + n->goff[L.pidx];
  if (pro) { a.in_scale = pro->scale; a.in_shift = pro->shift; a.in_relu = 1; }
  a.N = N; a.H = H; a.W = W; a.C = L.cin; a.K = L.cout; a.R = L.k; a.S = L.k; a.stride = L.stride; a.pad = L.pad; a.OH = OH; a.OW = OW;
  a.seg_images = seg_images; a.seg_stride = seg_stride;
  if (kind < 0 || !c->use_wg || c->prof.on) {
    TRY(prof_wgrad(c, c->dtype, a, st));
    return 0;
  }
  if (!c->wg_stream) {
    TRY(hipStreamCreateWithFlags(&c->wg_stream, hipStreamNonBlocking));
    for (int k = 0; k < 3; ++k) {
      TRY(hipEventCreateWithFlags(&c->ev_wg_in[k], hipEventDisableTiming));
      TRY(hipEventCreateWithFlags(&c->ev_wg_done[k], hipEventDisableTiming));
    }
    TRY(hipEventCreateWithFlags(&c->ev_wg_join, hipEventDisableTiming));
  }
  TRY(hipEventRecord(c->ev_wg_in[kind], st));
  TRY(hipStreamWaitEvent(c->wg_stream, c->ev_wg_in[kind], 0));
  TRY(prof_wgrad(c, c->dtype, a, c->wg_stream));
  TRY(hipEventRecord(c->ev_wg_done[kind], c->wg_stream));
  c->wg_pending[kind] = true;
  c->wg_any = true;
  return 0;
}

int launch_bucket_allreduce(sslcr_net* n, int bucket, size_t lo, size_t hi, hipStream_t st) {
  sslcr_ctx* c = n->ctx;
  if (!sharded(c) || hi <= lo) return 0;
  TRY(hipEventRecord(c->ev_ready[bucket], st));
  TRY(hipStreamWaitEvent(c->comm_stream, c->ev_ready[bucket], 0));
  TRYI(wg_join(c, c->comm_stream));
  float* g = (float*)n->grads.p + lo;
  TRYI(all_reduce(c, 1, g, hi - lo, false, c->comm_stream));
  return 0;
}

int lowest_trainable(const sslcr_net* n) {
  for (int i = 0; i < 60; ++i)
    if (n->rg[i]) return i;
  return 60;
}

int backbone_backward(sslcr_net* n, int npass, hipStream_t st) {
  sslcr_ctx* c = n->ctx;
  const int dt = c->dtype;
  const size_t es = c->esz();
  PassState* P = n->pass;
  const int N = P[0].N;
  const Dims d = make_dims(P[0].H, P[0].W);
  const int low = lowest_trainable(n);
  if (low >= 60) return 0;
  const size_t unit = (((size_t)N * d.ph * d.pw * 64 * es) + 255) & ~(size_t)255;
  const size_t stem_sz = (((size_t)N * d.oh0 * d.ow0 * 64 * es) + 255) & ~(size_t)255;
  TRYI(c->scratch.ensure(7 * npass * unit + stem_sz));
  char* S = (char*)c->scratch.p;
  auto buf = [&](int kind, int p, size_t bytes) { return S + (size_t)kind * npass * unit + (size_t)p * bytes; };
  int kOut = 0, kXin = 5;
  const int kG = 1, kRaw2 = 2, kAct1 = 3, kRaw1 = 4, kRawD = 6;
  char* dRaw0 = S + (size_t)7 * npass * unit;
  auto tap = [&](int blk, int slot, const void* src, int n_, int h_, int w_, int c_) -> int {
    if (!n->tap) return 0;
    const size_t bytes = (size_t)n_ * h_ * w_ * c_ * es;
    TRYI(n->tapbuf[blk][slot].ensure(bytes));
    TRY(hipMemcpyAsync(n->tapbuf[blk][slot].p, src, bytes, hipMemcpyDeviceToDevice, st));
    int* d4 = n->tapdims[blk][slot];
    d4[0] = n_; d4[1] = h_; d4[2] = w_; d4[3] = c_;
    return 0;
  };

  size_t hi_pending = n->goff[60];
  int bucket = 1;
  for (int p = 0; p < npass; ++p)
    TRY(launch_avgpool_bwd(dt, n->dE[p], buf(kOut, p, (size_t)N * d.lh[7] * d.lw[7] * 512 * es), N, d.lh[7] * d.lw[7], 512, st));
  for (int i = 7; i >= 0; --i) {
    BlockL& B = n->blocks[i];
    const int oh = d.lh[i], ow = d.lw[i];
    const int xh = i == 0 ? d.ph : d.lh[i - 1], xw = i == 0 ? d.pw : d.lw[i - 1];
    const size_t opix = (size_t)N * oh * ow;
    const bool need_dx = low < B.pstart;
    const size_t so = opix * B.c2.cout * es, si = (size_t)N * xh * xw * B.c1.cin * es;
    bool c2_batched = false;
    if (npass > 1) {
      WgradArgs q;
      memset(&q, 0, sizeof(q));
      q.N = N * npass; q.H = oh; q.W = ow; q.C = B.c2.cin; q.K = B.c2.cout; q.R = 3; q.S = 3; q.stride = 1; q.pad = 1; q.OH = oh; q.OW = ow;
      c2_batched = wgrad_halo_tw(q) != 0 && (wgrad_halo_tw(q) == 16 || N % 2 == 0);
    }
    ConvArgs seg_m;
    bool seg_dg = false;
    if (npass > 1 && segments_on() && !c->prof.on) {
      seg_m = conv_args(B.c2, nullptr, B.c2.w_dg, nullptr, N * npass, oh, ow);
      seg_m.C = B.c2.cout; seg_m.K = B.c2.cin; seg_m.transposed = 0; seg_m.PH = oh; seg_m.PW = ow; seg_m.OH = oh; seg_m.OW = ow;
      const BnSaved& s1 = P[0].bn[B.b1.bidx];
      seg_m.mask_x = P[0].blk[i].raw1; seg_m.mask_scale = s1.scale; seg_m.mask_shift = s1.shift; seg_m.mask_mean = s1.mean;
      seg_m.seg_images = N; seg_m.seg_stride = (int)(P[1].bn[B.b1.bidx].scale - s1.scale);
      seg_dg = conv_h16_ok(dt, seg_m) && conv_segments_ok(dt, seg_m) && conv_partials_rows(seg_m) % npass == 0;
    }
    const bool seg_bn = npass > 1 && segments_on() && !c->prof.on && !(sharded(c) && c->bn_sync) && c->bn_ring.p &&
                        c->bn_ring_i + 2 * npass <= sslcr_ctx::kBnRing;
    const int bn_stride = npass > 1 ? (int)(P[1].bn[0].scale - P[0].bn[0].scale) : 0;
    if (seg_bn) {
      char *dOut = buf(kOut, 0, so), *G = buf(kG, 0, so), *dRaw2 = buf(kRaw2, 0, so), *dRawD = buf(kRawD, 0, so);
      TRYI(wg_wait(c, 0, st));
      if (B.has_ds) TRYI(wg_wait(c, 2, st));
      const size_t apix = opix * npass;
      if (B.has_ds) {
        BnBwdArgs a2, ad;
        double* sums_2 = take_sums_n(c, npass);
        if (!sums_2) return fail("backbone_backward: ring slots");
        TRYI(bn_bwd_begin(n, B.b2, P[0].bn[B.b2.bidx], dOut, P[0].blk[i].raw2, P[0].blk[i].y, 0, dRaw2, G, apix, (double)opix, st, sums_2, &a2, nullptr, 1,
                          nullptr, 0, true, npass, bn_stride));
        TRYI(bn_bwd_begin(n, B.bd, P[0].bn[B.bd.bidx], G, P[0].blk[i].rawd, nullptr, 0, dRawD, nullptr, apix, (double)opix, st, sums_2 + 2 * B.b2.C, &ad,
                          nullptr, 0, nullptr, 0, true, npass, bn_stride));
        TRYI(bn_bwd_end(c, a2, st));
        TRYI(bn_bwd_end(c, ad, st));
      } else {
        TRYI(bn_backward(n, B.b2, P[0].bn[B.b2.bidx], dOut, P[0].blk[i].raw2, P[0].blk[i].y, 0, dRaw2, G, apix, (double)opix, st, nullptr, 1, nullptr, 0,
                         npass, bn_stride));
      }
      TRYI(tap(i, 0, G, N, oh, ow, B.c2.cout));
      TRYI(tap(i, 1, dRaw2, N, oh, ow, B.c2.cout));
      if (B.has_ds) TRYI(tap(i, 4, dRawD, N, oh, ow, B.ds.cout));
    }
    for (int p = 0; p < npass; ++p) {
      PassState& ps = P[p];
      char *dOut = buf(kOut, p, so), *G = buf(kG, p, so), *dRaw2 = buf(kRaw2, p, so), *dAct1 = buf(kAct1, p, so), *dRaw1 = buf(kRaw1, p, so),
           *dRawD = buf(kRawD, p, so);
      if (!seg_bn) {
      TRYI(wg_wait(c, 0, st));
      if (B.has_ds) TRYI(wg_wait(c, 2, st));
      if (B.has_ds) {
        BnBwdArgs a2, ad;
        double* ring = take_sums(c);
        double* sums_2 = ring ? ring : c->bn_sums;
        double* sums_d = sums_2 + 2 * B.b2.C;
        TRYI(bn_bwd_begin(n, B.b2, ps.bn[B.b2.bidx], dOut, ps.blk[i].raw2, ps.blk[i].y, 0, dRaw2, G, opix, (double)opix, st, sums_2, &a2, nullptr, 1,
                          nullptr, 0, ring != nullptr, 1, 0, true));
        TRYI(bn_bwd_begin(n, B.bd, ps.bn[B.bd.bidx], G, ps.blk[i].rawd, nullptr, 0, dRawD, nullptr, opix, (double)opix, st, sums_d, &ad, nullptr, 0,
                          nullptr, 0, ring != nullptr, 1, 0, true));
        const bool pair = bn_bwd_pair_ok(a2, ad);
        static const bool g_free = [] { const char* e = getenv("SSLCR_BN_PAIR_G"); return e && atoi(e) == 0; }();
        const int keep_g = (n->tap || !a2.yact_bits || !g_free) ? 1 : 0;
        if (pair) {
          TRY(launch_bn_bwd_reduce_pair(dt, a2, ad, keep_g, st));
        } else {
          TRY(launch_bn_bwd_reduce(dt, a2, st));
          TRY(launch_bn_bwd_reduce(dt, ad, st));
        }
        TRYI(bn_bwd_sync(c, sums_2, 4 * (size_t)B.b2.C, st));
        if (pair) {
          if (c->prof.on) {
            ProfRec r;
            r.e0 = c->prof.get(); r.e1 = c->prof.get();
            r.name = dt == DT_BF16 ? "sslcr::bn_bwd_apply_pair_kernel<unsigned short>" : "sslcr::bn_bwd_apply_pair_kernel<float>";
            r.flops = 0.0;
            r.bytes = (keep_g ? 5.0 : 5.0625) * (double)opix * B.b2.C * c->esz();
            (void)hipEventRecord(r.e0, st);
            hipError_t e = launch_bn_bwd_apply_pair(dt, a2, ad, keep_g, st);
            (void)hipEventRecord(r.e1, st);
            c->prof.rec[2].push_back(r);
            TRY(e);
          } else {
            TRY(launch_bn_bwd_apply_pair(dt, a2, ad, keep_g, st));
          }
        } else {
          TRYI(bn_bwd_end(c, a2, st));
          TRYI(bn_bwd_end(c, ad, st));
        }
      } else {
        TRYI(bn_backward(n, B.b2, ps.bn[B.b2.bidx], dOut, ps.blk[i].raw2, ps.blk[i].y, 0, dRaw2, G, opix, (double)opix, st, nullptr, 1));
      }
      if (p == 0) {
        TRYI(tap(i, 0, G, N, oh, ow, B.c2.cout));
        TRYI(tap(i, 1, dRaw2, N, oh, ow, B.c2.cout));
        if (B.has_ds) TRYI(tap(i, 4, dRawD, N, oh, ow, B.ds.cout));
      }
      }
      if (!c2_batched) TRYI(wgrad_call(n, B.c2, ps.blk[i].raw1, dRaw2, &ps.bn[B.b1.bidx], N, oh, ow, oh, ow, st, 0, 0, 0));
      if (seg_dg) continue;
      float* b1_rows = nullptr;
      int b1_nrows = 0;
      {
        ConvArgs a = conv_args(B.c2, dRaw2, B.c2.w_dg, dAct1, N, oh, ow);
        a.C = B.c2.cout; a.K = B.c2.cin; a.transposed = 0; a.PH = oh; a.PW = ow; a.OH = oh; a.OW = ow;
        ConvArgs m = a;
        const BnSaved& s1 = ps.bn[B.b1.bidx];
        m.mask_x = ps.blk[i].raw1; m.mask_scale = s1.scale; m.mask_shift = s1.shift; m.mask_mean = s1.mean;
        if (conv_h16_ok(dt, m)) {
          TRYI(ensure_partials(c, m, &b1_rows, &b1_nrows));
          m.stats = b1_rows;
          a = m;
        }
        TRY(prof_conv(c, dt,a, st));
        if (p == 0) {
          TRYI(tap(i, 2, dAct1, N, oh, ow, B.c2.cin));
          n->tap_flags[i] = b1_rows ? 1 : 0;
        }
      }
      TRYI(wg_wait(c, 1, st));
      TRYI(bn_backward(n, B.b1, ps.bn[B.b1.bidx], dAct1, ps.blk[i].raw1, nullptr, b1_rows ? 0 : 1, dRaw1, nullptr, opix, (double)opix, st,
                       nullptr, 0, b1_rows, b1_nrows));
      if (p == 0) TRYI(tap(i, 3, dRaw1, N, oh, ow, B.c1.cout));
    }
    if (seg_dg) {
      float* rows = nullptr;
      int nrows = 0;
      seg_m.x = buf(kRaw2, 0, so); seg_m.y = buf(kAct1, 0, so);
      TRYI(ensure_partials(c, seg_m, &rows, &nrows));
      seg_m.stats = rows;
      TRY(prof_conv(c, dt, seg_m, st));
      TRYI(tap(i, 2, buf(kAct1, 0, so), N, oh, ow, B.c2.cin));
      n->tap_flags[i] = 1;
      const int per = nrows / npass;
      if (seg_bn) {
        TRYI(wg_wait(c, 1, st));
        TRYI(bn_backward(n, B.b1, P[0].bn[B.b1.bidx], buf(kAct1, 0, so), P[0].blk[i].raw1, nullptr, 0, buf(kRaw1, 0, so), nullptr, opix * npass,
                         (double)opix, st, nullptr, 0, rows, nrows, npass, bn_stride));
        TRYI(tap(i, 3, buf(kRaw1, 0, so), N, oh, ow, B.c1.cout));
      }
      for (int p = 0; p < npass && !seg_bn; ++p) {
        PassState& ps = P[p];
        TRYI(wg_wait(c, 1, st));
        TRYI(bn_backward(n, B.b1, ps.bn[B.b1.bidx], buf(kAct1, p, so), ps.blk[i].raw1, nullptr, 0, buf(kRaw1, p, so), nullptr, opix, (double)opix, st,
                         nullptr, 0, rows + (size_t)p * per * 2 * B.b1.C, per));
        if (p == 0) TRYI(tap(i, 3, buf(kRaw1, 0, so), N, oh, ow, B.c1.cout));
      }
    }
    if (c2_batched)
      TRYI(wgrad_call(n, B.c2, P[0].blk[i].raw1, buf(kRaw2, 0, so), &P[0].bn[B.b1.bidx], N * npass, oh, ow, oh, ow, st, N,
                      (int)(P[1].bn[B.b1.bidx].scale - P[0].bn[B.b1.bidx].scale), 0));
    {
      const char* X0 = i == 0 ? P[0].pooled : P[0].blk[i - 1].y;
      TRYI(wgrad_call(n, B.c1, X0, buf(kRaw1, 0, so), nullptr, N * npass, xh, xw, oh, ow, st, 0, 0, 1));
      if (B.has_ds) TRYI(wgrad_call(n, B.ds, X0, buf(kRawD, 0, so), nullptr, N * npass, xh, xw, oh, ow, st, 0, 0, 2));
    }
    if (need_dx) {
      {
        const int NB = N * npass;
        char *G = buf(kG, 0, so), *dRaw1 = buf(kRaw1, 0, so), *dXin = buf(kXin, 0, si), *dRawD = buf(kRawD, 0, so);
        ConvArgs a = conv_args(B.c1, dRaw1, B.c1.w_dg, dXin, NB, oh, ow);
        a.C = B.c1.cout; a.K = B.c1.cin; a.transposed = (B.c1.stride == 1) ? 0 : 1; a.PH = xh; a.PW = xw; a.OH = xh; a.OW = xw;
        if (!B.has_ds) a.residual = G;
        if (B.c1.stride == 1) {
          TRY(prof_conv(c, dt,a, st));
        } else {
          ConvArgs q4 = a;
          q4.pix_mul = 2; q4.PH = xh / 2; q4.PW = xw / 2; q4.par4 = 1;
          const bool one = xh % 2 == 0 && xw % 2 == 0 && conv_dma_bp(dt, q4) != 0 && conv_dma_bp(DT_BF16, q4) == conv_dma_bp(dt, q4) &&
                           conv_halo_tw(dt, q4) == 0;
          if (one) TRY(prof_conv(c, dt, q4, st));
          for (int par = 0; par < (one ? 0 : 4); ++par) {
            ConvArgs q = a;
            const int ph_ = par >> 1, pw_ = par & 1;
            q.pix_mul = 2; q.pix_off_h = ph_; q.pix_off_w = pw_;
            q.PH = (xh - ph_ + 1) / 2; q.PW = (xw - pw_ + 1) / 2;
            if (q.PH <= 0 || q.PW <= 0) continue;
            unsigned m = 0;
            for (int r = 0; r < 3; ++r)
              for (int s2 = 0; s2 < 3; ++s2)
                if (((ph_ + 1 - r) & 1) == 0 && ((pw_ + 1 - s2) & 1) == 0) m |= 1u << (r * 3 + s2);
            q.tap_mask = m;
            TRY(prof_conv(c, dt,q, st));
          }
        }
        if (B.has_ds) {
          ConvArgs s = conv_args(B.ds, dRawD, B.ds.w_dg, dXin, NB, oh, ow);
          s.C = B.ds.cout; s.K = B.ds.cin; s.stride = 1; s.pad = 0; s.PH = oh; s.PW = ow; s.OH = xh; s.OW = xw; s.osh = B.ds.stride;
          s.accumulate = 1;
          TRY(prof_conv(c, dt,s, st));
        }
        TRYI(tap(i, 5, dXin, N, xh, xw, B.c1.cin));
      }
      const int t = kOut; kOut = kXin; kXin = t;
    }
    if (i == 6 || i == 4 || i == 2) {
      TRYI(launch_bucket_allreduce(n, bucket++, n->goff[B.pstart], hi_pending, st));
      hi_pending = n->goff[B.pstart];
    }
    if (!need_dx) break;
  }
  if (low < 3) {
    for (int p = 0; p < npass; ++p) {
      PassState& ps = P[p];
      PoolSrc pool{buf(kOut, p, (size_t)N * d.ph * d.pw * 64 * es), ps.argmax, d.oh0, d.ow0, d.ph, d.pw, ps.pooled};
      const size_t spix = (size_t)N * d.oh0 * d.ow0;
      StemWgradArgs w;
      memset(&w, 0, sizeof(w));
      w.x = ps.x; w.x2 = ps.x2; w.n_split = ps.n_split; w.dy = dRaw0; w.dw = (float*)n->grads.p + n->goff[0];
      w.N = N; w.H = ps.H; w.W = ps.W; w.OH = d.oh0; w.OW = d.ow0; w.in_f32 = ps.in_f32;
      if (n->rg[0] && c->fuse_stem_bwd) {
        BnBwdArgs a;
        double* ring = take_sums(c);
        double* sums0 = ring ? ring : c->bn_sums;
        TRYI(bn_bwd_begin(n, n->bn0, ps.bn[0], nullptr, ps.raw0, nullptr, 1, nullptr, nullptr, spix, (double)spix, st, sums0, &a, &pool, 0, nullptr, 0,
                          ring != nullptr));
        TRYI(bn_bwd_sync(c, sums0, 2 * 64, st));
        w.dy = nullptr;
        if (c->prof.on) {
          ProfRec r;
          r.e0 = c->prof.get(); r.e1 = c->prof.get();
          r.name = dt == DT_BF16 ? "sslcr::stem_wgrad_kernel<unsigned short, pool>" : "sslcr::stem_wgrad_kernel<float, pool>";
          r.flops = 0.0;
          const double t = (double)spix * 64 * c->esz();
          r.bytes = 0.25 * t + 0.25 * (double)spix * 64 + t + (double)N * 3 * ps.H * ps.W * (ps.in_f32 ? 4 : 1);
          (void)hipEventRecord(r.e0, st);
          hipError_t e = launch_stem_wgrad_pool(dt, w, a, st);
          (void)hipEventRecord(r.e1, st);
          c->prof.rec[2].push_back(r);
          TRY(e);
        } else {
          TRY(launch_stem_wgrad_pool(dt, w, a, st));
// ... 572 lines not shown
```

### ssl_cr_histo_amd/csrc/kernels.hpp

```cpp
#pragma once
#include "common.hpp"
#include "../../include/sslcr.h"

namespace sslcr {

using ConvArgs = sslcr_conv_desc;
using WgradArgs = sslcr_wgrad_desc;
using StemArgs = sslcr_stem_desc;
using StemWgradArgs = sslcr_stem_wgrad_desc;
using BnFinalizeArgs = sslcr_bn_finalize_desc;
using BnActArgs = sslcr_bn_act_desc;
using PoolFwdArgs = sslcr_pool_fwd_desc;
using PoolBwdArgs = sslcr_pool_bwd_desc;
using BnBwdArgs = sslcr_bn_bwd_desc;
using LossArgs = sslcr_loss_desc;
using TensorDesc = sslcr_tensor_desc;
using OptArgs = sslcr_opt_desc;
using PackArgs = sslcr_pack_desc;
using Fp8Args = sslcr_fp8_desc;
using PackFp8Args = sslcr_pack_fp8_desc;

hipError_t launch_conv(int dtype, const ConvArgs& a, hipStream_t st);
int conv_tile_bp(const ConvArgs& a);
const char* conv_kernel_name(int dtype, const ConvArgs& a);
const char* wgrad_kernel_name(int dtype, const WgradArgs& a);
int conv_partials_rows(const ConvArgs& a);
bool conv_segments_ok(int dtype, const ConvArgs& a);
int device_cus();
int conv_halo_tw(int dtype, const ConvArgs& a);
int conv_halo_tiles(const ConvArgs& a, int tw);
hipError_t launch_conv_halo(int dtype, const ConvArgs& a, int tw, hipStream_t st);
int conv_halo256_mode(int dtype, const ConvArgs& a);
int conv_halo256_tiles(const ConvArgs& a, int mode);
hipError_t launch_conv_halo256(int dtype, const ConvArgs& a, int mode, hipStream_t st);
bool conv_h16_ok(int dtype, const ConvArgs& a);
int conv_h16_rows(const ConvArgs& a);
hipError_t launch_conv_h16(int dtype, const ConvArgs& a, hipStream_t st);
const char* conv_h16_name(int dtype, const ConvArgs& a);
bool conv_pp64_ok(int dtype, const ConvArgs& a);
hipError_t launch_conv_pp64(const ConvArgs& a, hipStream_t st);
const char* conv_pp64_name(const ConvArgs& a);
int conv_pp64_rows(const ConvArgs& a);
int conv_dma_bp(int dtype, const ConvArgs& a);
int conv_dma_rows(const ConvArgs& a, int bp);
hipError_t launch_conv_dma(int dtype, const ConvArgs& a, int bp, hipStream_t st);
const char* conv_dma_name(int dtype, int bp);
bool conv_s2_ok(int dtype, const ConvArgs& a);
bool conv_s2_pair_ok(int dtype, const ConvArgs& a, const ConvArgs& d);
int conv_s2_rows(const ConvArgs& a);
hipError_t launch_conv_s2(const ConvArgs& a, const ConvArgs* d, hipStream_t st);
const char* conv_s2_name(const ConvArgs& a, bool pair);
bool conv_s2d_ok(int dtype, const ConvArgs& a);
hipError_t launch_conv_s2d(const ConvArgs& a, hipStream_t st);
const char* conv_s2d_name();
int conv_fp8_mode(const ConvArgs& a);
int conv_fp8_rows(const ConvArgs& a);
const char* conv_fp8_name(const ConvArgs& a);
hipError_t launch_conv_fp8(const ConvArgs& a, const Fp8Args& q, hipStream_t st);
hipError_t launch_pack_fp8(const PackFp8Args& a, hipStream_t st);
hipError_t launch_fp8_scale_update(float* slots, int n, hipStream_t st);
hipError_t launch_wgrad(int dtype, const WgradArgs& a, hipStream_t st);
int wgrad_halo_tw(const WgradArgs& a);
void* stream_scratch(hipStream_t st, size_t bytes);
void stream_scratch_release();
hipError_t launch_wgrad_fold(const void* slabs, float* dw, int C, int gx, int gy, int splits, int taps, int kh_n, hipStream_t st);
hipError_t launch_stem_wgrad_fold(const void* slabs, float* dw, int nwg, hipStream_t st);
hipError_t launch_wgrad_halo(int dtype, const WgradArgs& a, int tw, hipStream_t st);
bool wgrad_dma_ok(int dtype, const WgradArgs& a, int splits);
bool wgrad_dma_used(int dtype, const WgradArgs& a);
hipError_t launch_wgrad_dma(const WgradArgs& a, int tw, int tps, int ntiles, int splits, void* slabs, hipStream_t st);
hipError_t launch_probe_tr16(const uint16_t* in, const int* byte_addr, uint16_t* out, hipStream_t st);
bool wgrad_s2_ok(int dtype, const WgradArgs& a);
hipError_t launch_wgrad_s2(const WgradArgs& a, hipStream_t st);
hipError_t launch_stem(int dtype, const StemArgs& a, hipStream_t st);
int stem_partials_rows(const StemArgs& a);
hipError_t launch_stem_wgrad(int dtype, const StemWgradArgs& a, hipStream_t st);
hipError_t launch_stem_wgrad_pool(int dtype, const StemWgradArgs& a, const sslcr_bn_bwd_desc& b, hipStream_t st);
bool stem_pool_ok(int dtype, const StemArgs& a, int POH, int POW);
hipError_t launch_stem_pool(int dtype, const StemArgs& a, int POH, int POW, hipStream_t st);
hipError_t launch_bn_finalize(const BnFinalizeArgs& a, hipStream_t st);
hipError_t launch_bn_act(int dtype, const BnActArgs& a, hipStream_t st);
hipError_t launch_bn_relu_maxpool(int dtype, const PoolFwdArgs& a, hipStream_t st);
hipError_t launch_maxpool_relu_bwd(int dtype, const PoolBwdArgs& a, hipStream_t st);
hipError_t launch_avgpool_fwd(int dtype, const void* x, float* y, int N, int HW, int C, hipStream_t st);
hipError_t launch_avgpool_bwd(int dtype, const float* dy, void* dx, int N, int HW, int C, hipStream_t st);
hipError_t launch_bn_bwd_reduce(int dtype, const BnBwdArgs& a, hipStream_t st);
hipError_t launch_bn_bwd_apply(int dtype, const BnBwdArgs& a, hipStream_t st);
bool bn_bwd_pair_ok(const BnBwdArgs& a, const BnBwdArgs& b);
hipError_t launch_bn_bwd_reduce_pair(int dtype, const BnBwdArgs& a, const BnBwdArgs& b, int keep_g, hipStream_t st);
hipError_t launch_bn_bwd_apply_pair(int dtype, const BnBwdArgs& a, const BnBwdArgs& b, int from_g, hipStream_t st);
hipError_t launch_bn_param_grads(const double* sums, const float* invstd, float* dgamma, float* dbeta, int C, hipStream_t st);
hipError_t launch_bn_param_grads_scaled(const double* sums, const float* invstd, float* dgamma, float* dbeta, int C, float scale, hipStream_t st);
hipError_t launch_linear_fwd(const float* x, const float* w, const float* b, float* y, int M, int N, int K, int relu, hipStream_t st);
hipError_t launch_linear_bwd(const float* x, const float* w, const float* dy, const float* yact, float* dx, float* dw, float* db,
                             int M, int N, int K, int dx_accumulate, float* scratch, hipStream_t st);
hipError_t launch_loss(const LossArgs& a, hipStream_t st);
hipError_t launch_softmax_col(const float* logits, float* out, int n, int C, int col, hipStream_t st);
hipError_t launch_weak_augment(const sslcr_weak_aug_desc& a, hipStream_t st);
hipError_t launch_hed_colour(const sslcr_colour_aug_desc& a, hipStream_t st);
hipError_t launch_brightness_contrast(const sslcr_brightness_contrast_desc& a, hipStream_t st);
hipError_t launch_optimizer(const TensorDesc* d_descs, int ntensors, int max_n, const OptArgs& o, hipStream_t st);
constexpr int OPT_CHUNK = 2048;
constexpr int OPT_TILE = 16 * 16 * 9;
hipError_t launch_optimizer_chunks(const TensorDesc* d_descs, const void* d_chunks , int nchunks,
                                   const OptArgs& o, hipStream_t st);
hipError_t launch_axpby(float* p, float* q, size_t n, float alpha, int copy_back, hipStream_t st);
hipError_t launch_fill(float* p, size_t n, float v, hipStream_t st);
hipError_t launch_pack_conv(int dtype, const PackArgs& a, hipStream_t st);
hipError_t launch_pack_stem(int dtype, const PackArgs& a, hipStream_t st);
hipError_t launch_copy2d(float* dst, long ldd, const float* src, long lds, int rows, int w, int accumulate, hipStream_t st);
// ... 8 lines not shown
```

### ssl_cr_histo_amd/kernels.py

```python
import torch

from . import _lib as L

F32, BF16 = 0, 1


def tdtype(dtype):
    return torch.bfloat16 if dtype == BF16 else torch.float32


def _dt(t):
    if t.dtype == torch.bfloat16:
        return BF16
    if t.dtype == torch.float32:
        return F32
    raise TypeError(f"unsupported activation dtype {t.dtype}")


def _chk(*ts):
    for t in ts:
        if t is not None:
            if not t.is_cuda:
                raise L.SslcrError("sslcr kernels need device tensors (no CPU fallback)")
            if not t.is_contiguous():
                raise L.SslcrError("sslcr kernels need contiguous tensors")


last_conv_kernel = ""
last_wgrad_kernel = ""


def conv2d(x, w, stride, pad, *, in_scale=None, in_shift=None, in_relu=False, bias=None, residual=None, relu=False,
           want_stats=False, out=None, transposed=False, out_hw=None, osh=1, accumulate=False, pixel_hw=None,
           pix_mul=0, pix_off=(0, 0), tap_mask=0, mask=None, par4=False, seg_images=0, out_scale=None):
    _chk(x, w, in_scale, in_shift, bias, residual, out, out_scale)
    dt = _dt(x)
    N, H, W, C = x.shape
    K, R, S, C2 = w.shape
    assert C2 == C and w.dtype == x.dtype
    if transposed:
        PH, PW = pixel_hw
    else:
        PH, PW = (H + 2 * pad - R) // stride + 1, (W + 2 * pad - S) // stride + 1
    OH, OW = out_hw if out_hw is not None else (PH * osh, PW * osh)
    y = out if out is not None else torch.empty((N, OH, OW, K), dtype=x.dtype, device=x.device)
    d = L.ConvDesc(L.ptr(x), L.ptr(w), L.ptr(y), L.ptr(in_scale), L.ptr(in_shift), L.ptr(bias), L.ptr(residual), None,
                   N, H, W, C, K, R, S, stride, pad, PH, PW, OH, OW, osh, int(transposed), int(in_relu), int(relu),
                   int(accumulate), int(pix_mul), int(pix_off[0]), int(pix_off[1]), int(tap_mask))
    d.par4 = int(par4)
    d.out_scale = L.ptr(out_scale)
    if seg_images:
        d.seg_images = int(seg_images)
        d.seg_stride = int(in_scale.stride(0)) if in_scale is not None and in_scale.dim() == 2 else 0
        if not L.lib().sslcr_conv2d_segments_ok(dt, d):
            raise L.SslcrError("conv2d: no segment form for this shape / dtype")
    if mask is not None:
        _chk(*mask)
        d.mask_x, d.mask_scale, d.mask_shift, d.mask_mean = (L.ptr(t) for t in mask)
    stats = None
    if want_stats:
        rows = L.lib().sslcr_conv2d_partial_rows(d)
        stats = torch.full((rows, 2, K), float("nan"), dtype=torch.float32, device=x.device)
        d.stats = L.ptr(stats)
    global last_conv_kernel
    last_conv_kernel = L.lib().sslcr_conv2d_kernel_name(dt, d).decode()
    L.check(L.lib().sslcr_conv2d(dt, d, L.stream_ptr()))
    return (y, stats) if want_stats else y


def conv2d_s2_pair(x, w3, w1, *, bias3=None, bias1=None, relu3=False, want_stats=False, scale3=None, scale1=None):
    _chk(x, w3, w1, bias3, bias1, scale3, scale1)
    dt = _dt(x)
    N, H, W, C = x.shape
    K = w3.shape[0]
    assert w3.shape == (K, 3, 3, C) and w1.shape == (K, 1, 1, C)
    PH, PW = H // 2, W // 2
    y3 = torch.empty((N, PH, PW, K), dtype=x.dtype, device=x.device)
    yd = torch.empty_like(y3)
    d3 = L.ConvDesc(L.ptr(x), L.ptr(w3), L.ptr(y3), None, None, L.ptr(bias3), None, None,
                    N, H, W, C, K, 3, 3, 2, 1, PH, PW, PH, PW, 1, 0, 0, int(relu3), 0, 0, 0, 0, 0)
    d1 = L.ConvDesc(L.ptr(x), L.ptr(w1), L.ptr(yd), None, None, L.ptr(bias1), None, None,
                    N, H, W, C, K, 1, 1, 2, 0, PH, PW, PH, PW, 1, 0, 0, 0, 0, 0, 0, 0, 0)
    d3.out_scale, d1.out_scale = L.ptr(scale3), L.ptr(scale1)
    s3 = sd = None
    if want_stats:
        rows = L.lib().sslcr_conv2d_partial_rows(d3)
        s3 = torch.full((rows, 2, K), float("nan"), dtype=torch.float32, device=x.device)
        sd = torch.full((rows, 2, K), float("nan"), dtype=torch.float32, device=x.device)
        d3.stats, d1.stats = L.ptr(s3), L.ptr(sd)
    if not L.lib().sslcr_conv2d_s2_pair_ok(dt, d3, d1):
        raise L.SslcrError("conv2d_s2_pair: not served")
    L.check(L.lib().sslcr_conv2d_s2_pair(dt, d3, d1, L.stream_ptr()))
    return (y3, yd, s3, sd) if want_stats else (y3, yd)


def pack_conv_fp8(w_kcrs, *, bn=None, eps=1e-5):
    _chk(w_kcrs)
    K, C, R, S = w_kcrs.shape
    assert R == 3 and S == 3
    dev = w_kcrs.device
    w8 = torch.empty((K, 3, 3, C), dtype=torch.uint8, device=dev)
    dq = torch.empty(K, dtype=torch.float32, device=dev)
    bias = torch.empty(K, dtype=torch.float32, device=dev) if bn is not None else None
    g, b, rm, rv = bn if bn is not None else (None, None, None, None)
    d = L.PackFp8Desc(L.ptr(w_kcrs), L.ptr(w8), L.ptr(dq), L.ptr(g), L.ptr(b), L.ptr(rm), L.ptr(rv), eps, L.ptr(bias), K, C)
    L.check(L.lib().sslcr_pack_conv_fp8(d, L.stream_ptr()))
    return w8, dq, bias


def conv2d_fp8(x, w8, w_dequant, *, x_scale=1.0, in_scale=None, in_shift=None, in_relu=False, bias=None, residual=None, relu=False,
               want_stats=False, amax_out=None):
    _chk(x, w8, w_dequant, in_scale, in_shift, bias, residual)
    assert x.dtype == torch.bfloat16 and w8.dtype == torch.uint8
    N, H, W, C = x.shape
    K = w8.shape[0]
    y = torch.empty((N, H, W, K), dtype=torch.bfloat16, device=x.device)
    d = L.ConvDesc(L.ptr(x), None, L.ptr(y), L.ptr(in_scale), L.ptr(in_shift), L.ptr(bias), L.ptr(residual), None,
                   N, H, W, C, K, 3, 3, 1, 1, H, W, H, W, 1, 0, int(in_relu), int(relu), 0, 0, 0, 0, 0)
    q = L.Fp8Desc(L.ptr(w8), L.ptr(w_dequant), float(x_scale), None, L.ptr(amax_out))
    stats = None
    if want_stats:
        rows = L.lib().sslcr_conv2d_fp8_partial_rows(d)
        stats = torch.full((rows, 2, K), float("nan"), dtype=torch.float32, device=x.device)
        d.stats = L.ptr(stats)
    L.check(L.lib().sslcr_conv2d_fp8(d, q, L.stream_ptr()))
    return (y, stats) if want_stats else y


def conv2d_wgrad(x, dy, dw, R, S, stride, pad, *, in_scale=None, in_shift=None, in_relu=False, seg_images=0):
    _chk(x, dy, dw, in_scale, in_shift)
    N, H, W, C = x.shape
    _, OH, OW, K = dy.shape
    assert dw.shape == (K, R, S, C) and dw.dtype == torch.float32
    d = L.WgradDesc(L.ptr(x), L.ptr(dy), L.ptr(dw), L.ptr(in_scale), L.ptr(in_shift), int(in_relu),
                    N, H, W, C, K, R, S, stride, pad, OH, OW, int(seg_images), C if seg_images else 0)
    global last_wgrad_kernel
    last_wgrad_kernel = L.lib().sslcr_conv2d_wgrad_kernel_name(_dt(x), d).decode()
    L.check(L.lib().sslcr_conv2d_wgrad(_dt(x), d, L.stream_ptr()))


def pack_conv(w_kcrs, dtype, *, fwd=True, dgrad=False, bn=None, eps=1e-5, dgrad_flip=False, unfold=False):
    _chk(w_kcrs)
    K, C, R, S = w_kcrs.shape
    dev = w_kcrs.device
    wf = torch.empty((K, R, S, C), dtype=tdtype(dtype), device=dev) if fwd else None
    wd = torch.empty((C, R, S, K), dtype=tdtype(dtype), device=dev) if dgrad else None
    bias = torch.empty(K, dtype=torch.float32, device=dev) if bn is not None else None
    g, b, rm, rv = bn if bn is not None else (None, None, None, None)
    scale = torch.empty(K, dtype=torch.float32, device=dev) if (unfold and bn is not None) else None
    d = L.PackDesc(L.ptr(w_kcrs), L.ptr(wf), L.ptr(wd), L.ptr(g), L.ptr(b), L.ptr(rm), L.ptr(rv), eps, L.ptr(bias),
# ... 241 lines not shown
```

Baseline: 69890.

## Save BN-applied conv2 input during forward to skip re-transform in wgrad

The conv2 forward kernels (h16 and pp64) now optionally write the BN+ReLU-transformed input tile (a1) they already hold in registers out to a side buffer with nontemporal stores. The backward weight-gradient for conv2 then reads this saved activation directly, with no in_scale/in_shift, instead of reapplying the batch-norm affine on raw1. This is enabled by default for blocks with C != 64 in bf16 non-fp8 mode. It trades extra forward write bandwidth and memory for a cheaper wgrad input path.

After: 70300, median of 6. Within noise of the previous version (+0.6%).

```diff
diff --git a/include/sslcr.h b/include/sslcr.h
--- a/include/sslcr.h
+++ b/include/sslcr.h
@@ -37,10 +37,12 @@
   int par4;
   int seg_images, seg_stride;
   const float* out_scale;
+  void* xf_out;
 } sslcr_conv_desc;
 int sslcr_conv2d(int dtype, const sslcr_conv_desc* d, void* stream);
 int sslcr_conv2d_partial_rows(const sslcr_conv_desc* d);
 int sslcr_conv2d_segments_ok(int dtype, const sslcr_conv_desc* d);
+int sslcr_conv2d_xf_out_ok(int dtype, const sslcr_conv_desc* d);
 const char* sslcr_conv2d_kernel_name(int dtype, const sslcr_conv_desc* d);
 int sslcr_conv2d_s2_pair(int dtype, const sslcr_conv_desc* c1, const sslcr_conv_desc* ds, void* stream);
 int sslcr_conv2d_s2_pair_ok(int dtype, const sslcr_conv_desc* c1, const sslcr_conv_desc* ds);
diff --git a/ssl_cr_histo_amd/_lib.py b/ssl_cr_histo_amd/_lib.py
--- a/ssl_cr_histo_amd/_lib.py
+++ b/ssl_cr_histo_amd/_lib.py
@@ -22,7 +22,7 @@
               [(k, i32) for k in ("N", "H", "W", "C", "K", "R", "S", "stride", "pad", "PH", "PW", "OH", "OW", "osh",
                                   "transposed", "in_relu", "relu", "accumulate", "pix_mul", "pix_off_h", "pix_off_w")] +
               [("tap_mask", C.c_uint), ("mask_x", vp), ("mask_scale", vp), ("mask_shift", vp), ("mask_mean", vp),
-               ("par4", i32), ("seg_images", i32), ("seg_stride", i32), ("out_scale", vp)])
+               ("par4", i32), ("seg_images", i32), ("seg_stride", i32), ("out_scale", vp), ("xf_out", vp)])
 WgradDesc = _S("WgradDesc", [("x", vp), ("dy", vp), ("dw", vp), ("in_scale", vp), ("in_shift", vp), ("in_relu", i32)] +
                [(k, i32) for k in ("N", "H", "W", "C", "K", "R", "S", "stride", "pad", "OH", "OW", "seg_images", "seg_stride")])
 StemDesc = _S("StemDesc", [("x", vp), ("w", vp), ("y", vp), ("bias", vp), ("stats", vp)] +
@@ -72,6 +72,7 @@
     "sslcr_conv2d": (i32, [i32, P(ConvDesc), vp]),
     "sslcr_conv2d_partial_rows": (i32, [P(ConvDesc)]),
     "sslcr_conv2d_segments_ok": (i32, [i32, P(ConvDesc)]),
+    "sslcr_conv2d_xf_out_ok": (i32, [i32, P(ConvDesc)]),
     "sslcr_conv2d_kernel_name": (C.c_char_p, [i32, P(ConvDesc)]),
     "sslcr_conv2d_s2_pair": (i32, [i32, P(ConvDesc), P(ConvDesc), vp]),
     "sslcr_conv2d_s2_pair_ok": (i32, [i32, P(ConvDesc), P(ConvDesc)]),
diff --git a/ssl_cr_histo_amd/csrc/capi.cpp b/ssl_cr_histo_amd/csrc/capi.cpp
--- a/ssl_cr_histo_amd/csrc/capi.cpp
+++ b/ssl_cr_histo_amd/csrc/capi.cpp
@@ -29,7 +29,7 @@
 
 extern "C" {
 
-int sslcr_version(void) { return 6; }
+int sslcr_version(void) { return 7; }
 const char* sslcr_last_error(void) { return g_err; }
 
 int sslcr_conv2d(int dtype, const sslcr_conv_desc* d, void* stream) {
@@ -40,10 +40,16 @@
   NEED(d->K % 64 == 0, "K % 64");
   NEED(d->osh >= 1 && d->PH > 0 && d->PW > 0, "pixel space");
   NEED(conv_segments_ok(dtype, *d), "seg_images: no segment form for this shape / dtype (sslcr_conv2d_segments_ok)");
+  if (d->xf_out) {
+    NEED(dtype == SSLCR_BF16 && d->in_scale && d->in_shift, "xf_out: bf16 with in_scale / in_shift only");
+    NEED((reinterpret_cast<uintptr_t>(d->xf_out) & 15) == 0, "xf_out must be 16-byte aligned");
+    NEED(conv_xf_out_ok(dtype, *d), "xf_out: the kernel serving this descriptor does not write it (sslcr_conv2d_xf_out_ok)");
+  }
   return check(launch_conv(dtype, *d, (hipStream_t)stream), "conv2d");
 }
 int sslcr_conv2d_partial_rows(const sslcr_conv_desc* d) { return d ? conv_partials_rows(*d) : -1; }
 int sslcr_conv2d_segments_ok(int dtype, const sslcr_conv_desc* d) { return (d && (dtype == DT_F32 || dtype == DT_BF16) && conv_segments_ok(dtype, *d)) ? 1 : 0; }
+int sslcr_conv2d_xf_out_ok(int dtype, const sslcr_conv_desc* d) { return (d && conv_xf_out_ok(dtype, *d)) ? 1 : 0; }
 const char* sslcr_conv2d_kernel_name(int dtype, const sslcr_conv_desc* d) { return d ? conv_kernel_name(dtype, *d) : ""; }
 int sslcr_conv2d_s2_pair_ok(int dtype, const sslcr_conv_desc* c1, const sslcr_conv_desc* ds) {
   return (c1 && ds && conv_s2_pair_ok(dtype, *c1, *ds)) ? 1 : 0;
@@ -58,6 +64,7 @@
 int sslcr_conv2d_fp8(const sslcr_conv_desc* d, const sslcr_fp8_desc* q, void* stream) {
   NEED(d && q && d->x && d->y && q->w8 && q->w_dequant, "null tensor");
   NEED(q->x_scale > 0.f, "x_scale must be positive");
+  NEED(!d->xf_out, "xf_out: not written by the fp8 kernel");
   NEED(conv_fp8_mode(*d) != 0, "shape not served by the fp8 kernel (3x3/1, C % 128, K % 128, 16x16-tileable or 8x8 with N % 4)");
   return check(launch_conv_fp8(*d, *q, (hipStream_t)stream), "conv2d_fp8");
 }
diff --git a/ssl_cr_histo_amd/csrc/common.hpp b/ssl_cr_histo_amd/csrc/common.hpp
--- a/ssl_cr_histo_amd/csrc/common.hpp
+++ b/ssl_cr_histo_amd/csrc/common.hpp
@@ -155,6 +155,11 @@
 __device__ __forceinline__ void st16(void* p, const u32x4_t& v) { *reinterpret_cast<u32x4_t*>(p) = v; }
 __device__ __forceinline__ u32x4_t ld16_nt(const void* p) { return __builtin_nontemporal_load(reinterpret_cast<const u32x4_t*>(p)); }
 __device__ __forceinline__ void st16_nt(void* p, const u32x4_t& v) { __builtin_nontemporal_store(v, reinterpret_cast<u32x4_t*>(p)); }
+#ifdef SSLCR_XF_OUT_PLAIN
+#define SSLCR_XF_ST(p, v) st16(p, v)
+#else
+#define SSLCR_XF_ST(p, v) st16_nt(p, v)
+#endif
 
 struct LdsDma {
 #if defined(__HIP_DEVICE_COMPILE__)
diff --git a/ssl_cr_histo_amd/csrc/conv_h16.hip b/ssl_cr_histo_amd/csrc/conv_h16.hip
--- a/ssl_cr_histo_amd/csrc/conv_h16.hip
+++ b/ssl_cr_histo_amd/csrc/conv_h16.hip
@@ -96,6 +96,7 @@
   t.x = reinterpret_cast<const char*>(a.x) + px * a.C * es;
   t.y = reinterpret_cast<char*>(a.y) + px * a.K * es;
   if (a.residual) t.residual = reinterpret_cast<const char*>(a.residual) + px * a.K * es;
+  if (a.xf_out) t.xf_out = reinterpret_cast<char*>(a.xf_out) + px * a.C * es;
   return t;
 }
 int conv_h16_rows(const ConvArgs& a) {
diff --git a/ssl_cr_histo_amd/csrc/conv_h16_body.hpp b/ssl_cr_histo_amd/csrc/conv_h16_body.hpp
--- a/ssl_cr_histo_amd/csrc/conv_h16_body.hpp
+++ b/ssl_cr_histo_amd/csrc/conv_h16_body.hpp
@@ -154,6 +154,16 @@
     for (int i = 0; i < NLD; ++i)
       if ((hvalid >> i) & 1u) st16(s_halo + st_off[i], hreg[i]);
   };
+  auto save_xf = [&](const Geo& q, int sl) {
+    if constexpr (XF && sizeof(T) == 2) {
+      if (a.xf_out && q.k0 == 0) {
+        char* xo = reinterpret_cast<char*>(a.xf_out) + ((size_t)sl * CE + chunk * EPC) * sizeof(T);
+#pragma unroll
+        for (int i = 0; i < NLD; ++i)
+          if (((hvalid >> i) & 1u) && !((edge >> (4 * i)) & 0xfull)) SSLCR_XF_ST(xo + (size_t)(q.origin + rel[i]) * a.C * sizeof(T), hreg[i]);
+      }
+    }
+  };
   LdsDma wdma;
   wdma.init(wg, 0x7fffffffu);
   auto dma_w = [&](int k0, int slab, int tap0, int half) {
@@ -199,6 +209,7 @@
 #pragma unroll
   for (int i = 0; i < NLD; ++i) xform_one(i);
   store_halo();
+  if constexpr (WR) save_xf(cur, 0);
   SSLCR_WAIT_VM0();
   __syncthreads();
   frags(0, 0, s_w);
@@ -276,6 +287,7 @@
         H16_T(tp2);
         H16_ACC(0, tp1 - tp0); H16_ACC(1, tp2 - tp1);
         if (i == 8) {
+          save_xf(cur, slab);
           load_res();
           load_halo(nxt, nslab);
           load_affine(nslab);
@@ -300,6 +312,9 @@
     wb ^= 1;
     frags(0, 0, WR ? s_w : s_w + wb * (TPB * WBUF));
     __builtin_amdgcn_sched_barrier(0);
+    if constexpr (WR) {
+      if (!done) save_xf(nxt, nslab);
+    }
 
     H16_T(te0);
     if (last) {
diff --git a/ssl_cr_histo_amd/csrc/conv_igemm.hip b/ssl_cr_histo_amd/csrc/conv_igemm.hip
--- a/ssl_cr_histo_amd/csrc/conv_igemm.hip
+++ b/ssl_cr_histo_amd/csrc/conv_igemm.hip
@@ -338,8 +338,16 @@
   return false;
 }
 
+bool conv_xf_out_ok(int dtype, const ConvArgs& a) {
+  if (dtype != DT_BF16 || a.residual || a.mask_x || a.out_scale || a.transposed || a.par4) return false;
+  ConvArgs q = a;
+  if (!q.in_scale) { static const float one = 1.f; q.in_scale = &one; q.in_shift = &one; }
+  return conv_segments_ok(dtype, q) && conv_h16_ok(dtype, q);
+}
+
 hipError_t launch_conv(int dtype, const ConvArgs& a, hipStream_t st) {
   if (!conv_segments_ok(dtype, a)) return hipErrorInvalidValue;
+  if (a.xf_out && (!a.in_scale || !conv_xf_out_ok(dtype, a))) return hipErrorInvalidValue;
   if (a.out_scale && (!a.bias || a.stats || a.mask_x)) return hipErrorInvalidValue;
   if (conv_h16_ok(dtype, a)) return launch_conv_h16(dtype, a, st);
   if (a.mask_x) return hipErrorInvalidValue;
diff --git a/ssl_cr_histo_amd/csrc/conv_pp64.hip b/ssl_cr_histo_amd/csrc/conv_pp64.hip
--- a/ssl_cr_histo_amd/csrc/conv_pp64.hip
+++ b/ssl_cr_histo_amd/csrc/conv_pp64.hip
@@ -142,7 +142,8 @@
       hin |= (ok ? 1u : 0u) << i;
     }
   };
-  auto xform_store = [&]() {
+  char* xo = XF ? reinterpret_cast<char*>(a.xf_out) + (size_t)chunk * EPC * sizeof(T) : nullptr;
+  auto xform_store = [&](const Geo& q, bool sv) {
     float sc[EPC], sh[EPC];
     if (XF) {
       const f32x4_t c0 = *reinterpret_cast<const f32x4_t*>(s_scale + chunk * EPC), c1 = *reinterpret_cast<const f32x4_t*>(s_scale + chunk * EPC + 4);
@@ -166,6 +167,10 @@
       int rl = role[i];
       asm volatile("" : "+v"(rl));
       if ((hvalid >> i) & 1u) st16(s_halo + ((rl >> 12) & 0xffff0), v);
+      if constexpr (XF) {
+        if (sv && ((hvalid >> i) & 1u) && !((edge >> (4 * i)) & 0xfull))
+          SSLCR_XF_ST(xo + (unsigned)(q.origin + (rl & 0xffff) - rel_bias) * (unsigned)(64 * sizeof(T)), v);
+      }
     }
   };
 
@@ -201,7 +206,7 @@
   load_halo(cur);
   __builtin_amdgcn_s_waitcnt(0x0f70);
   SSLCR_PP_BAR();
-  xform_store();
+  xform_store(cur, XF && live && a.xf_out != nullptr);
   Geo nxt = geom(tile_of(1, live_n));
   load_halo(nxt);
   SSLCR_PP_BAR();
@@ -240,7 +245,7 @@
     PP_ACC(0, t1 - t0); PP_ACC(1, t2 - t1);
 
     load_res(cur);
-    xform_store();
+    xform_store(nxt, XF && live_n && a.xf_out != nullptr);
     PP_T(ta);
     PP_ACC(4, ta - t2);
     {
diff --git a/ssl_cr_histo_amd/csrc/engine.cpp b/ssl_cr_histo_amd/csrc/engine.cpp
--- a/ssl_cr_histo_amd/csrc/engine.cpp
+++ b/ssl_cr_histo_amd/csrc/engine.cpp
@@ -98,6 +98,8 @@
   struct {
     char *raw1, *raw2, *rawd, *y;
     uint8_t* ybits;
+    char* a1;
+    bool a1_ok;
   } blk[8];
   BnSaved bn[20];
   float* E = nullptr;
@@ -292,7 +294,7 @@
   const double M = (double)a.N * a.PH * a.PW;
   const double src = (double)a.N * a.H * a.W;
   r.flops = a.transposed ? 2.0 * src * a.C * a.K * rs : 2.0 * M * a.K * a.C * rs;
-  r.bytes = (src * a.C + (double)a.K * rs * a.C + M * a.K * (a.residual ? 2.0 : 1.0) * (a.accumulate ? 2.0 : 1.0)) * es;
+  r.bytes = (src * a.C * (a.xf_out ? 2.0 : 1.0) + (double)a.K * rs * a.C + M * a.K * (a.residual ? 2.0 : 1.0) * (a.accumulate ? 2.0 : 1.0)) * es;
   r.name = conv_kernel_name(dt, a);
   (void)hipEventRecord(r.e0, st);
   hipError_t e = launch_conv(dt, a, st);
@@ -623,6 +625,12 @@
   return d;
 }
 
+bool save_a1_wanted(const sslcr_ctx* c, int C) {
+  static const int mode = [] { const char* e = getenv("SSLCR_SAVE_A1"); return e ? atoi(e) : 1; }();
+  if (c->dtype != DT_BF16 || c->fp8) return false;
+  return mode == 2 || (mode != 0 && C != 64);
+}
+
 int alloc_passes(sslcr_net* n, int npass, int N, int H, int W) {
   const size_t es = n->ctx->esz();
   const Dims d = make_dims(H, W);
@@ -630,13 +638,14 @@
   auto take = [&](size_t per_pass) { return c.take(per_pass * npass); };
   const size_t s_raw0 = (size_t)N * d.oh0 * d.ow0 * 64 * es, s_pool = (size_t)N * d.ph * d.pw * 64 * es, s_arg = (size_t)N * d.ph * d.pw * 64;
   const size_t o_raw0 = take(s_raw0), o_pool = take(s_pool), o_arg = take(s_arg);
-  size_t o_blk[8][4], s_blk[8], o_bits[8], s_bits[8];
+  size_t o_blk[8][4], s_blk[8], o_bits[8], s_bits[8], o_a1[8];
   bool bits_ok = true;
   for (int i = 0; i < 8; ++i) {
     s_blk[i] = (size_t)N * d.lh[i] * d.lw[i] * kBlockCfg[i][1] * es;
     for (int j = 0; j < 4; ++j) o_blk[i][j] = (j == 2 && !n->blocks[i].has_ds) ? 0 : take(s_blk[i]);
     s_bits[i] = (((size_t)N * d.lh[i] * d.lw[i] * kBlockCfg[i][1] / 8) + 127) / 128 * 128;
     o_bits[i] = take(s_bits[i]);
+    o_a1[i] = save_a1_wanted(n->ctx, kBlockCfg[i][1]) ? take(s_blk[i]) : 0;
     if (s_bits[i] * 8 != (size_t)N * d.lh[i] * d.lw[i] * kBlockCfg[i][1]) bits_ok = false;
   }
   const size_t s_bn = 20 * 4 * 512 * sizeof(float), s_E = (size_t)N * 512 * sizeof(float);
@@ -651,6 +660,8 @@
       ps.blk[i].rawd = n->blocks[i].has_ds ? b + o_blk[i][2] + p * s_blk[i] : nullptr;
       ps.blk[i].y = b + o_blk[i][3] + p * s_blk[i];
       ps.blk[i].ybits = (uint8_t*)(b + o_bits[i] + p * s_bits[i]);
+      ps.blk[i].a1 = save_a1_wanted(n->ctx, kBlockCfg[i][1]) ? b + o_a1[i] + p * s_blk[i] : nullptr;
+      ps.blk[i].a1_ok = false;
     }
     float* f = (float*)(b + o_bn + p * s_bn);
     for (int i = 0; i < 20; ++i) {
@@ -754,6 +765,9 @@
     if (segs) { a2.seg_images = N; a2.seg_stride = seg_stride; }
     TRYI(ensure_partials(c, a2, &part, &rows, !segs && use_fp8(c, B.c2, a2)));
     a2.stats = part;
+    const bool keep = ps.blk[i].a1 && save_a1_wanted(c, a2.C) && !use_fp8(c, B.c2, a2) && conv_xf_out_ok(dt, a2);
+    if (keep) a2.xf_out = ps.blk[i].a1;
+    for (int p = 0; p < nseg; ++p) (&ps)[p].blk[i].a1_ok = keep;
     TRY(segs ? prof_conv(c, dt, a2, st) : prof_conv_fwd(c, dt, a2, B.c2, false, st));
     TRYI(finalize_bn(n, B.b2, part, rows, cnt, ps.bn[B.b2.bidx], replay, st, nseg, seg_stride));
     BnActArgs e;
@@ -1181,6 +1195,8 @@
     const size_t opix = (size_t)N * oh * ow;
     const bool need_dx = low < B.pstart;
     const size_t so = opix * B.c2.cout * es, si = (size_t)N * xh * xw * B.c1.cin * es;
+    bool a1w = true;
+    for (int p = 0; p < npass; ++p) a1w = a1w && P[p].blk[i].a1 && P[p].blk[i].a1_ok;
     bool c2_batched = false;
     if (npass > 1) {
       WgradArgs q;
@@ -1278,7 +1294,7 @@
         if (B.has_ds) TRYI(tap(i, 4, dRawD, N, oh, ow, B.ds.cout));
       }
       }
-      if (!c2_batched) TRYI(wgrad_call(n, B.c2, ps.blk[i].raw1, dRaw2, &ps.bn[B.b1.bidx], N, oh, ow, oh, ow, st, 0, 0, 0));
+      if (!c2_batched) TRYI(wgrad_call(n, B.c2, a1w ? ps.blk[i].a1 : ps.blk[i].raw1, dRaw2, a1w ? nullptr : &ps.bn[B.b1.bidx], N, oh, ow, oh, ow, st, 0, 0, 0));
       if (seg_dg) continue;
       float* b1_rows = nullptr;
       int b1_nrows = 0;
@@ -1328,7 +1344,9 @@
         if (p == 0) TRYI(tap(i, 3, buf(kRaw1, 0, so), N, oh, ow, B.c1.cout));
       }
     }
-    if (c2_batched)
+    if (c2_batched && a1w)
+      TRYI(wgrad_call(n, B.c2, P[0].blk[i].a1, buf(kRaw2, 0, so), nullptr, N * npass, oh, ow, oh, ow, st, 0, 0, 0));
+    else if (c2_batched)
       TRYI(wgrad_call(n, B.c2, P[0].blk[i].raw1, buf(kRaw2, 0, so), &P[0].bn[B.b1.bidx], N * npass, oh, ow, oh, ow, st, N,
                       (int)(P[1].bn[B.b1.bidx].scale - P[0].bn[B.b1.bidx].scale), 0));
     {
diff --git a/ssl_cr_histo_amd/csrc/kernels.hpp b/ssl_cr_histo_amd/csrc/kernels.hpp
--- a/ssl_cr_histo_amd/csrc/kernels.hpp
+++ b/ssl_cr_histo_amd/csrc/kernels.hpp
@@ -26,6 +26,7 @@
 const char* wgrad_kernel_name(int dtype, const WgradArgs& a);
 int conv_partials_rows(const ConvArgs& a);
 bool conv_segments_ok(int dtype, const ConvArgs& a);
+bool conv_xf_out_ok(int dtype, const ConvArgs& a);
 int device_cus();
 int conv_halo_tw(int dtype, const ConvArgs& a);
 int conv_halo_tiles(const ConvArgs& a, int tw);
diff --git a/ssl_cr_histo_amd/kernels.py b/ssl_cr_histo_amd/kernels.py
--- a/ssl_cr_histo_amd/kernels.py
+++ b/ssl_cr_histo_amd/kernels.py
@@ -32,8 +32,8 @@
 
 def conv2d(x, w, stride, pad, *, in_scale=None, in_shift=None, in_relu=False, bias=None, residual=None, relu=False,
            want_stats=False, out=None, transposed=False, out_hw=None, osh=1, accumulate=False, pixel_hw=None,
-           pix_mul=0, pix_off=(0, 0), tap_mask=0, mask=None, par4=False, seg_images=0, out_scale=None):
-    _chk(x, w, in_scale, in_shift, bias, residual, out, out_scale)
+           pix_mul=0, pix_off=(0, 0), tap_mask=0, mask=None, par4=False, seg_images=0, out_scale=None, xf_out=None):
+    _chk(x, w, in_scale, in_shift, bias, residual, out, out_scale, xf_out)
     dt = _dt(x)
     N, H, W, C = x.shape
     K, R, S, C2 = w.shape
@@ -49,6 +49,9 @@
                    int(accumulate), int(pix_mul), int(pix_off[0]), int(pix_off[1]), int(tap_mask))
     d.par4 = int(par4)
     d.out_scale = L.ptr(out_scale)
+    if xf_out is not None:
+        assert xf_out.shape == x.shape and xf_out.dtype == x.dtype
+        d.xf_out = L.ptr(xf_out)
     if seg_images:
         d.seg_images = int(seg_images)
         d.seg_stride = int(in_scale.stride(0)) if in_scale is not None and in_scale.dim() == 2 else 0
@@ -66,6 +69,13 @@
     last_conv_kernel = L.lib().sslcr_conv2d_kernel_name(dt, d).decode()
     L.check(L.lib().sslcr_conv2d(dt, d, L.stream_ptr()))
     return (y, stats) if want_stats else y
+
+
+def conv2d_xf_out_ok(dtype, N, H, W, C, K, *, R=3, S=3, stride=1, pad=1, seg_images=0):
+    PH, PW = (H + 2 * pad - R) // stride + 1, (W + 2 * pad - S) // stride + 1
+    d = L.ConvDesc(None, None, None, None, None, None, None, None, N, H, W, C, K, R, S, stride, pad, PH, PW, PH, PW, 1, 0, 1, 0, 0, 0, 0, 0, 0)
+    d.seg_images = int(seg_images)
+    return bool(L.lib().sslcr_conv2d_xf_out_ok(dtype, d))
 
 
 def conv2d_s2_pair(x, w3, w1, *, bias3=None, bias1=None, relu3=False, want_stats=False, scale3=None, scale1=None):
```
